# wyhlovecpp/GPT-Image-Edit

Measured on AMD Instinct MI355X. Metric: edited images/sec, 28-step FLUX-Kontext (VAE encode + 28 x MMDiT + VAE decode), higher is better.
Workload: dtype bf16; 1 GPU; cfg2_single_512x512_28step; batch_per_gpu=1, global_batch=1, height=512, width=512, S_txt=512, S_tgt=1024, S_cond=1024, seq_len=2560, num_inference_steps=28, blocks=19 double + 38 single, parallelism=dp1

## Files before the change

### gpt_image_edit_amd/csrc/gemm_epilogue.h

```cpp
#pragma once

#include "mxfp8_quant.h"

constexpr int BM = 256;

struct TileRows {
  int ld, wrap, rpb, b0, r0;
  float inv;
  bool big;
  FK_DEV TileRows(const fk_rows& r, int m0) {
    ld = (int)r.ld;
    if (r.rows_per_batch <= 0) { rpb = 0x7fffffff; wrap = 0; b0 = 0; r0 = 0; big = true; inv = 0.f; }
    else {
      rpb = (int)(r.rows_per_batch > 0x7fffffff ? 0x7fffffff : r.rows_per_batch);
      b0 = (unsigned)m0 / (unsigned)rpb;
      r0 = m0 - b0 * rpb;
      wrap = (int)(r.batch_stride - (int64_t)rpb * r.ld);
      big = rpb >= BM;
      inv = 1.0f / (float)rpb;
    }
  }
  FK_DEV int crossed(int ml) const {
    const int r = r0 + ml;
    const int one = r >= rpb ? 1 : 0;
    const int many = (int)(((float)r + 0.5f) * inv);
    return big ? one : many;
  }
  FK_DEV int off(int ml) const { return ml * ld + crossed(ml) * wrap; }
};

template <int N>
FK_DEV float row_ror(float v) {
  return __int_as_float(__builtin_amdgcn_update_dpp(0, __float_as_int(v), 0x120 + N, 0xf, 0xf, false));
}
FK_DEV float row16_sum(float v) {
  v += row_ror<8>(v);
  v += row_ror<4>(v);
  v += row_ror<2>(v);
  v += row_ror<1>(v);
  return v;
}

FK_DEV int xcd_chunk_index() {
  const int nwg = gridDim.x;
  const int q = nwg >> 3, r = nwg & 7;
  const int xcd = blockIdx.x & 7, idx = blockIdx.x >> 3;
  return (xcd < r ? xcd * (q + 1) : r * (q + 1) + (xcd - r) * q) + idx;
}

template <bool M16>
struct FragMap {
  static FK_DEV int row(int lane, int q) { return M16 ? (q & 1) * 16 + (lane & 15) : (lane & 31); }
  static FK_DEV int col(int lane, int q) { return M16 ? (q >> 1) * 16 + (lane >> 4) * 4 : 8 * q + 4 * (lane >> 5); }
};
FK_DEV f32x4_t quad_get(const f32x16_t& v, int q) { return f32x4_t{v[4 * q], v[4 * q + 1], v[4 * q + 2], v[4 * q + 3]}; }
FK_DEV void quad_set(f32x16_t& v, int q, const f32x4_t& c) {
  v[4 * q] = c[0]; v[4 * q + 1] = c[1]; v[4 * q + 2] = c[2]; v[4 * q + 3] = c[3];
}

template <int EPI, int BN, class C, int HALF = -1, int UB = 8>
FK_DEV void store_tile(const f32x16_t (&acc)[C::NF][C::MF], const fk_gemm_args& p, char* smem, int m0, int n0,
                       int wm, int wn, const u32x4_t* other = nullptr) {
  constexpr int MF0 = HALF > 0 ? C::MF / 2 : 0, MF1 = HALF == 0 ? C::MF / 2 : C::MF;
  constexpr int row0 = HALF > 0 ? BM / 2 : 0;
  int tid = threadIdx.x;
  if constexpr (C::NTHREADS == 256) asm volatile("" : "+v"(tid));
  const int lane = tid & 63;
  using FM = FragMap<C::M16>;
  u32x2_t bw[C::NF][4];
#pragma unroll
  for (int nf = 0; nf < C::NF; ++nf)
#pragma unroll
    for (int q = 0; q < 4; ++q) bw[nf][q] = u32x2_t{0u, 0u};
  if constexpr (EPI != FK_EPI_SCALE) {
    if (p.bias) {
#pragma unroll
      for (int nf = 0; nf < C::NF; ++nf)
#pragma unroll
        for (int q = 0; q < 4; ++q) {
          const int n = n0 + C::tile_col(wn, nf) + FM::col(lane, q);
          bw[nf][q] = *(const u32x2_t*)((const bf16_t*)p.bias + min(n, p.N - 4));
        }
    }
  }
  if constexpr (EPI == FK_EPI_F32DBG) {
#pragma unroll
    for (int nf = 0; nf < C::NF; ++nf)
#pragma unroll
      for (int q = 0; q < 4; ++q) {
        const int n = n0 + C::tile_col(wn, nf) + FM::col(lane, q);
        const float b[4] = {bf_lo(bw[nf][q][0]), bf_hi(bw[nf][q][0]), bf_lo(bw[nf][q][1]), bf_hi(bw[nf][q][1])};
#pragma unroll
        for (int mf = MF0; mf < MF1; ++mf) {
          const int m = m0 + C::tile_row(wm, mf) + FM::row(lane, q);
          f32x4_t x = quad_get(acc[nf][mf], q);
          if constexpr (HALF >= 0) {
#pragma unroll
            for (int j = 0; j < 4; ++j) x[j] += __uint_as_float(other[nf * 2 * C::MF + (mf - MF0) * 4 + q][j]);
          }
          if (m < p.M && n < p.N)
            *(f32x4_t*)((float*)p.C + fk_row_offset(p.c, m) + n) = f32x4_t{x[0] + b[0], x[1] + b[1], x[2] + b[2], x[3] + b[3]};
        }
      }
    return;
  }
  __syncthreads();
  bf16_t* ct = (bf16_t*)smem;
#pragma unroll
  for (int nf = 0; nf < C::NF; ++nf) {
#pragma unroll
    for (int q = 0; q < 4; ++q) {
      const int nl = C::tile_col(wn, nf) + FM::col(lane, q);
      const float b[4] = {bf_lo(bw[nf][q][0]), bf_hi(bw[nf][q][0]), bf_lo(bw[nf][q][1]), bf_hi(bw[nf][q][1])};
#pragma unroll
      for (int mf = MF0; mf < MF1; ++mf) {
        float v[4];
#pragma unroll
        for (int j = 0; j < 4; ++j) {
          float x = acc[nf][mf][q * 4 + j];
          if constexpr (HALF >= 0) x += __uint_as_float(other[nf * 2 * C::MF + (mf - MF0) * 4 + q][j]);
          if constexpr (EPI == FK_EPI_SCALE) v[j] = x * p.alpha;
          else v[j] = x + b[j];
        }
        if constexpr (EPI == FK_EPI_GELU_TANH || EPI == FK_EPI_SILU) {
          round_bf_pair(v[0], v[1]);
          round_bf_pair(v[2], v[3]);
#pragma unroll
          for (int j = 0; j < 4; ++j) v[j] = EPI == FK_EPI_GELU_TANH ? gelu_tanh_f(v[j]) : silu_f(v[j]);
        }
        u32x2_t pk;
        pk[0] = pack_bf2(v[0], v[1]);
        pk[1] = pack_bf2(v[2], v[3]);
        const int ml = C::tile_row(wm, mf) + FM::row(lane, q);
        *(u32x2_t*)(ct + ml * C::CT_LD + nl) = pk;
      }
    }
  }
  __syncthreads();
  constexpr int CPR = BN / 8;
  constexpr int ITERS = (HALF >= 0 ? BM / 2 : BM) * CPR / C::NTHREADS;
  constexpr int U = (EPI == FK_EPI_QKV && (ITERS > 8 || HALF >= 0)) ? 4 : UB;
  static_assert(ITERS % U == 0 && C::NTHREADS % CPR == 0, "epilogue batching");
  const TileRows crow(p.c, m0);
  bf16_t* const cbase = (bf16_t*)p.C + fk_row_offset(p.c, m0);
  const TileRows rrow = (EPI == FK_EPI_GATE_RES || EPI == FK_EPI_RES) ? TileRows(p.r, m0) : crow;
  const bf16_t* const rbase =
      (EPI == FK_EPI_GATE_RES || EPI == FK_EPI_RES) ? (const bf16_t*)p.res + fk_row_offset(p.r, m0) : nullptr;
  fk_rows gr = {0, 0, 0};
  if constexpr (EPI == FK_EPI_GATE_RES) gr.rows_per_batch = p.gate_rows_per_batch;
  const TileRows grow(gr, m0);
  const int D = EPI == FK_EPI_QKV ? p.qkv_heads * 128 : 1;
  const int which = EPI == FK_EPI_QKV ? n0 / D : 0;
  const int cc = tid % CPR, ml0 = row0 + tid / CPR;
  constexpr int ML_STEP = C::NTHREADS / CPR;
  const int n = n0 + cc * 8;
  const int nc = min(n, p.N - 8);
  const int mlast = p.M - 1 - m0;

  if (EPI == FK_EPI_QKV && which < 2) {
    const int hn = n - which * D;
    const int head = hn >> 7, dch = hn & 127;
    const u32x4_t ww = *(const u32x4_t*)((const bf16_t*)(which == 0 ? p.wq : p.wk) + dch);
    bf16_t* const dst = (bf16_t*)(which == 0 ? p.q_out : p.k_out);
#pragma unroll
    for (int j0 = 0; j0 < ITERS; j0 += U) {
      u32x4_t y[U];
      f32x4_t t0[U], t1[U];
      int srow[U], bidx[U];
#pragma unroll
      for (int u = 0; u < U; ++u) {
        const int ml = ml0 + ML_STEP * (j0 + u);
        y[u] = *(const u32x4_t*)(ct + ml * C::CT_LD + cc * 8);
        const int mlc = min(ml, mlast);
        const int nb = crow.crossed(mlc);
        bidx[u] = crow.b0 + nb;
        srow[u] = p.qkv_s_offset + crow.r0 + mlc - nb * crow.rpb;
        const float* tp = p.rope_cs + (int64_t)srow[u] * 128 + dch;
        t0[u] = *(const f32x4_t*)tp;
        t1[u] = *(const f32x4_t*)(tp + 4);
      }
#pragma unroll
      for (int u = 0; u < U; ++u) {
        const int ml = ml0 + ML_STEP * (j0 + u);
        float xv[8];
        float ss = 0.f;
#pragma unroll
        for (int e = 0; e < 4; ++e) {
          xv[2 * e] = bf_lo(y[u][e]);
          xv[2 * e + 1] = bf_hi(y[u][e]);
          ss += xv[2 * e] * xv[2 * e] + xv[2 * e + 1] * xv[2 * e + 1];
        }
        ss = row16_sum(ss);
        const float rs = __builtin_amdgcn_rsqf(ss * (1.0f / 128) + 1e-6f);
        const float cs[4] = {t0[u][0], t0[u][2], t1[u][0], t1[u][2]};
        const float sn[4] = {t0[u][1], t0[u][3], t1[u][1], t1[u][3]};
        u32x4_t ow;
#pragma unroll
        for (int e = 0; e < 4; ++e) {
          float re = xv[2 * e] * rs, im = xv[2 * e + 1] * rs;
          round_bf_pair(re, im);
          re *= bf_lo(ww[e]);
          im *= bf_hi(ww[e]);
          round_bf_pair(re, im);
          const float o0 = __fadd_rn(__fmul_rn(re, cs[e]), __fmul_rn(-im, sn[e]));
          const float o1 = __fadd_rn(__fmul_rn(im, cs[e]), __fmul_rn(re, sn[e]));
          ow[e] = pack_bf2(o0, o1);
        }
        const int hrow = (bidx[u] * p.qkv_heads + head) * p.qkv_s_total + srow[u];
        if (ml <= mlast && n < p.N) *(u32x4_t*)(dst + (int64_t)hrow * 128 + dch) = ow;
      }
    }
    return;
  }

#pragma unroll
  for (int j0 = 0; j0 < ITERS; j0 += U) {
    u32x4_t y[U], rv[U], gv[U];
    int coff[U];
#pragma unroll
    for (int u = 0; u < U; ++u) {
      const int ml = ml0 + ML_STEP * (j0 + u);
      const int mlc = min(ml, mlast);
      y[u] = *(const u32x4_t*)(ct + ml * C::CT_LD + cc * 8);
      coff[u] = crow.off(mlc) + n;
      if constexpr (EPI == FK_EPI_GATE_RES || EPI == FK_EPI_RES) rv[u] = *(const u32x4_t*)(rbase + rrow.off(mlc) + nc);
      if constexpr (EPI == FK_EPI_GATE_RES) {
        const int64_t b = grow.b0 + grow.crossed(mlc);
        gv[u] = *(const u32x4_t*)((const bf16_t*)p.gate + b * p.gate_batch_stride + nc);
      }
    }
#pragma unroll
    for (int u = 0; u < U; ++u) {
      const int ml = ml0 + ML_STEP * (j0 + u);
      u32x4_t o = y[u];
      if constexpr (EPI == FK_EPI_GATE_RES || EPI == FK_EPI_RES) {
#pragma unroll
        for (int e = 0; e < 4; ++e) {
          float y0 = bf_lo(o[e]), y1 = bf_hi(o[e]);
          if constexpr (EPI == FK_EPI_GATE_RES) {
            y0 *= bf_lo(gv[u][e]);
            y1 *= bf_hi(gv[u][e]);
            round_bf_pair(y0, y1);
          }
          o[e] = pack_bf2(bf_lo(rv[u][e]) + y0, bf_hi(rv[u][e]) + y1);
        }
      }
      if (ml <= mlast && n < p.N) *(u32x4_t*)(cbase + coff[u]) = o;
    }
  }
}

template <int EPI, int BN, class C>
FK_DEV void store_tile_mxq(const f32x16_t (&acc)[C::NF][C::MF], const fk_gemm_args& p, uint8_t* __restrict__ q,
                           uint8_t* __restrict__ s, int64_t ldq, int64_t ld_scale, char* smem, int m0, int n0, int wm, int wn) {
  static_assert(EPI == FK_EPI_NONE || EPI == FK_EPI_GELU_TANH, "quantized output: plain and GELU epilogues");
  const int tid = threadIdx.x, lane = tid & 63;
  using FM = FragMap<C::M16>;
  u32x2_t bw[C::NF][4];
#pragma unroll
  for (int nf = 0; nf < C::NF; ++nf)
#pragma unroll
    for (int qd = 0; qd < 4; ++qd) bw[nf][qd] = u32x2_t{0u, 0u};
  if (p.bias) {
#pragma unroll
    for (int nf = 0; nf < C::NF; ++nf)
#pragma unroll
      for (int qd = 0; qd < 4; ++qd) {
        const int n = n0 + C::tile_col(wn, nf) + FM::col(lane, qd);
        bw[nf][qd] = *(const u32x2_t*)((const bf16_t*)p.bias + min(n, p.N - 4));
      }
  }
  __syncthreads();
  bf16_t* ct = (bf16_t*)smem;
#pragma unroll
  for (int nf = 0; nf < C::NF; ++nf) {
#pragma unroll
    for (int qd = 0; qd < 4; ++qd) {
      const int nl = C::tile_col(wn, nf) + FM::col(lane, qd);
      const float b[4] = {bf_lo(bw[nf][qd][0]), bf_hi(bw[nf][qd][0]), bf_lo(bw[nf][qd][1]), bf_hi(bw[nf][qd][1])};
#pragma unroll
      for (int mf = 0; mf < C::MF; ++mf) {
        float v[4];
#pragma unroll
        for (int j = 0; j < 4; ++j) v[j] = acc[nf][mf][qd * 4 + j] + b[j];
        if constexpr (EPI == FK_EPI_GELU_TANH) {
          round_bf_pair(v[0], v[1]);
          round_bf_pair(v[2], v[3]);
#pragma unroll
          for (int j = 0; j < 4; ++j) v[j] = gelu_tanh_f(v[j]);
        }
        u32x2_t pk;
        pk[0] = pack_bf2(v[0], v[1]);
        pk[1] = pack_bf2(v[2], v[3]);
        const int ml = C::tile_row(wm, mf) + FM::row(lane, qd);
        *(u32x2_t*)(ct + ml * C::CT_LD + nl) = pk;
      }
    }
  }
  __syncthreads();
  constexpr int BPR = BN / 32;
  constexpr int ITERS = BM * BPR / C::NTHREADS;
  constexpr int ML_STEP = C::NTHREADS / BPR;
  static_assert(C::NTHREADS % BPR == 0 && (BM * BPR) % C::NTHREADS == 0, "quantized epilogue tiling");
  const int bc = tid % BPR, ml0 = tid / BPR;
  const int mlast = p.M - 1 - m0;
#pragma unroll
  for (int j = 0; j < ITERS; ++j) {
    const int ml = ml0 + ML_STEP * j;
    const u32x4_t* src = (const u32x4_t*)(ct + ml * C::CT_LD + bc * 32);
    uint32_t w[16], out[8];
#pragma unroll
    for (int i = 0; i < 4; ++i) {
      const u32x4_t v = src[i];
      w[4 * i] = v[0]; w[4 * i + 1] = v[1]; w[4 * i + 2] = v[2]; w[4 * i + 3] = v[3];
    }
    const uint32_t sbyte = mx_quant_block(w, out);
    if (ml <= mlast) {
      const int64_t m = (int64_t)m0 + ml;
      u32x4_t* dst = (u32x4_t*)(q + m * ldq + n0 + bc * 32);
      dst[0] = u32x4_t{out[0], out[1], out[2], out[3]};
      dst[1] = u32x4_t{out[4], out[5], out[6], out[7]};
      s[m * ld_scale + (n0 >> 5) + bc] = (uint8_t)sbyte;
    }
  }
}
```

### gpt_image_edit_amd/csrc/gemm_pingpong_bf16.hip

```cpp
#include <stdlib.h>

#include <type_traits>

#include "fk_common.h"

namespace {

#include "gemm_epilogue.h"
#ifndef FK_GROUP_M
#define FK_GROUP_M 8
#endif
constexpr int GROUP_M = FK_GROUP_M;
#ifndef FK_RATE_256
#define FK_RATE_256 1.22
#endif


enum { SK_WHOLE = 0, SK_SYM = 1, SK_SYM_UNANNOUNCED = 2 };

struct GroupArgs {
  fk_gemm_args p[FK_MAX_GROUP];
  int tiles_before[FK_MAX_GROUP + 1];
  int n;
  int big_cols;
  int small_before[FK_MAX_GROUP + 1];
  int xcd_big_start[8], xcd_big_cnt[8], xcd_small_start[8];
  float* sk_partials;
  unsigned* sk_ctl;
  int sk_mode;
  int sk_min_part;
  int group_m;
};

typedef __attribute__((address_space(3))) void lds_void;
typedef __attribute__((address_space(1))) const void gbl_void;

typedef short s16x4_t __attribute__((ext_vector_type(4)));
FK_DEV s16x4_t lds_tr16(const char* p) {
  return __builtin_amdgcn_ds_read_tr16_b64_v4i16((__attribute__((address_space(3))) s16x4_t*)p);
}

FK_DEV void buffer_lds16(__amdgpu_buffer_rsrc_t rsrc, char* lds_dst, int voffset, int soffset) {
#if defined(__HIP_DEVICE_COMPILE__)
  __builtin_amdgcn_raw_ptr_buffer_load_lds(rsrc, (lds_void*)lds_dst, 16, voffset, soffset, 0, 0);
#else
  (void)rsrc; (void)lds_dst; (void)voffset; (void)soffset;
#endif
}

FK_DEV void buffer_lds16(const BufDesc& d, char* lds_dst, int voffset, int soffset) {
  buffer_lds_opaque<16>(d, lds_addr_of(lds_dst), voffset, soffset);
}

template <int N>
FK_DEV void wait_vmcnt() {
  if constexpr (N == 0) asm volatile("s_waitcnt vmcnt(0)" ::: "memory");
  else if constexpr (N == 2) asm volatile("s_waitcnt vmcnt(2)" ::: "memory");
  else if constexpr (N == 4) asm volatile("s_waitcnt vmcnt(4)" ::: "memory");
  else if constexpr (N == 6) asm volatile("s_waitcnt vmcnt(6)" ::: "memory");
  else if constexpr (N == 8) asm volatile("s_waitcnt vmcnt(8)" ::: "memory");
  else if constexpr (N == 10) asm volatile("s_waitcnt vmcnt(10)" ::: "memory");
  else if constexpr (N == 12) asm volatile("s_waitcnt vmcnt(12)" ::: "memory");
  else static_assert(N == 0, "add the vmcnt literal");
}


template <int BN>
FK_DEV void tile_of(const GroupArgs& ga, const int (&before)[FK_MAX_GROUP + 1], int t, int nbn, int col0, int& pi, int& m0,
                    int& n0) {
  pi = 0;
#pragma unroll
  for (int i = 1; i < FK_MAX_GROUP; ++i)
    if (i < ga.n && t >= before[i]) pi = i;
  const fk_gemm_args& p = ga.p[pi];
  t -= before[pi];
  const int nbm = (p.M + BM - 1) / BM;
  const int per_group = ga.group_m * nbn;
  const int g = t / per_group;
  const int first_m = g * ga.group_m;
  const int gm = min(nbm - first_m, ga.group_m);
  const int rem = t - g * per_group;
  m0 = (first_m + rem % gm) * BM;
  n0 = col0 + (rem / gm) * BN;
}
template <int BN>
FK_DEV void select_tile(const GroupArgs& ga, int t, int& pi, int& m0, int& n0) {
  tile_of<BN>(ga, ga.tiles_before, t, (ga.p[0].N + BN - 1) / BN, 0, pi, m0, n0);
}

FK_DEV void mma16_block(f32x16_t& blk, const bf16x8_t& w0, const bf16x8_t& w1, const bf16x8_t& a0, const bf16x8_t& a1) {
  quad_set(blk, 0, __builtin_amdgcn_mfma_f32_16x16x32_bf16(w0, a0, quad_get(blk, 0), 0, 0, 0));
  quad_set(blk, 2, __builtin_amdgcn_mfma_f32_16x16x32_bf16(w1, a0, quad_get(blk, 2), 0, 0, 0));
  quad_set(blk, 1, __builtin_amdgcn_mfma_f32_16x16x32_bf16(w0, a1, quad_get(blk, 1), 0, 0, 0));
  quad_set(blk, 3, __builtin_amdgcn_mfma_f32_16x16x32_bf16(w1, a1, quad_get(blk, 3), 0, 0, 0));
}



template <int BN, bool M16_ = false>
struct Cfg8 {
  static_assert(BN == 256, "the ping-pong kernel is instantiated for the 256 x 256 tile only");
  static constexpr bool M16 = M16_;
  static constexpr int NTHREADS = 512;
  static constexpr int BK = 64, ROW_BYTES = 128;
  static constexpr int WAVES_M = 2, WAVES_N = 4;
  static constexpr int MF = 4, NF = 2;
  static constexpr int HALF_BYTES = 128 * ROW_BYTES;
  static constexpr int BUF_BYTES = 4 * HALF_BYTES;
  static constexpr int RING_BYTES = 2 * BUF_BYTES;
  static constexpr int CT_LD = BN + 8;
  static constexpr int CT_BYTES = BM * CT_LD * 2;
  static constexpr int SMEM_BYTES = RING_BYTES > CT_BYTES ? RING_BYTES : CT_BYTES;
  static FK_DEV int swz(int row) { return (row >> 1) & 7; }
  static FK_DEV int tile_row(int wm, int mf) { return (mf >> 1) * 128 + wm * 64 + (mf & 1) * 32; }
  static FK_DEV int tile_col(int wn, int nf) { return nf * 128 + wn * 32; }
};

template <int EPI, int BN, int LAY = 0, bool M16 = false, bool SYM = false>
FK_DEV void gemm8_body(const GroupArgs& ga, char* smem, int pi, int m0, int n0, int kt_first, int nk, int sk_slot, int sk_part = 0) {
  using C = Cfg8<BN, M16>;
  constexpr bool AT = LAY == 2, WT = LAY >= 1;
  const int tid = threadIdx.x;
  const int lane = tid & 63;
  const int wave = __builtin_amdgcn_readfirstlane(tid >> 6);
  const int wm = wave >> 2, wn = wave & 3;
  const fk_gemm_args& p = ga.p[pi];
  const int kbase = kt_first * (C::BK * 2);

  const int lrow = lane >> 3, slot = lane & 7;
  const int prow = lane >> 4, pslot = lane & 15;
  const __amdgpu_buffer_rsrc_t rs_a = __builtin_amdgcn_make_buffer_rsrc(
      (void*)((const bf16_t*)p.A + (AT ? (int64_t)m0 : fk_row_offset(p.a, m0))), 0, 0x7fffffff, 0x00020000);
  const __amdgpu_buffer_rsrc_t rs_w = __builtin_amdgcn_make_buffer_rsrc(
      (void*)((const bf16_t*)p.W + (WT ? (int64_t)n0 : (int64_t)n0 * p.ldw)), 0, 0x7fffffff, 0x00020000);
  const BufDesc od_a = make_buf_desc((const bf16_t*)p.A + (AT ? (int64_t)m0 : fk_row_offset(p.a, m0)), 0x7fffffffu);
  const BufDesc od_w = make_buf_desc((const bf16_t*)p.W + (WT ? (int64_t)n0 : (int64_t)n0 * p.ldw), 0x7fffffffu);
  int a_voff[2][2], w_voff[2][2];
  {
    const TileRows arow(p.a, m0);
    const int ldw2 = (int)p.ldw * 2, lda2 = (int)p.a.ld * 2;
#pragma unroll
    for (int h = 0; h < 2; ++h)
#pragma unroll
      for (int j = 0; j < 2; ++j) {
        const int rl = h * 128 + (wave * 2 + j) * 8 + lrow;
        const int sw = (slot ^ C::swz(rl)) << 4;
        const int kl = (wave * 2 + j) * 4 + prow;
        const int ct = (h * 128 + (((((pslot >> 2) ^ prow) << 2) | (pslot & 3)) << 3)) * 2;
        a_voff[h][j] = AT ? kl * lda2 + ct : arow.off(min(rl, p.M - 1 - m0)) * 2 + sw;
        w_voff[h][j] = WT ? kl * ldw2 + ct : min(rl, p.N - 1 - n0) * ldw2 + sw;
      }
  }
  const int kstep_a = AT ? C::BK * (int)p.a.ld * 2 : C::BK * 2, kstep_w = WT ? C::BK * (int)p.ldw * 2 : C::BK * 2;
  auto dma_half = [&](int which, int buf, int kt) {
    const int ktc = min(kt, nk - 1);
    char* dst = smem + buf * C::BUF_BYTES + which * C::HALF_BYTES + wave * 2048;
    if (which < 2) {
      const int koff = (AT ? 0 : kbase) + ktc * kstep_a;
      if constexpr (AT || WT) {
        buffer_lds16(od_a, dst, a_voff[which][0], koff);
        buffer_lds16(od_a, dst + 1024, a_voff[which][1], koff);
      } else {
        buffer_lds16(rs_a, dst, a_voff[which][0], koff);
        buffer_lds16(rs_a, dst + 1024, a_voff[which][1], koff);
      }
    } else {
      const int koff = (WT ? 0 : kbase) + ktc * kstep_w;
      if constexpr (AT || WT) {
        buffer_lds16(od_w, dst, w_voff[which - 2][0], koff);
        buffer_lds16(od_w, dst + 1024, w_voff[which - 2][1], koff);
      } else {
        buffer_lds16(rs_w, dst, w_voff[which - 2][0], koff);
        buffer_lds16(rs_w, dst + 1024, w_voff[which - 2][1], koff);
      }
    }
  };

  constexpr int NKS = M16 ? 2 : 4;
  constexpr int ASUB = M16 ? 4 : 2;
  constexpr int WSUB = M16 ? 2 : 1;
  constexpr int SUB_BYTES = (M16 ? 16 : 32) * C::ROW_BYTES;
  const int frow = M16 ? (lane & 15) : (lane & 31), fhalf = M16 ? (lane >> 4) : (lane >> 5), fsw = C::swz(frow);
  int koffs[NKS];
#pragma unroll
  for (int kk = 0; kk < NKS; ++kk) koffs[kk] = ((kk * (M16 ? 4 : 2) + fhalf) ^ fsw) << 4;
  const int a_rd = (wm * 64 + frow) * C::ROW_BYTES;
  const int w_rd = (wn * 32 + frow) * C::ROW_BYTES;

  f32x16_t acc[C::NF][C::MF];
#pragma unroll
  for (int i = 0; i < C::NF; ++i)
#pragma unroll
    for (int j = 0; j < C::MF; ++j)
#pragma unroll
      for (int r = 0; r < 16; ++r) acc[i][j][r] = 0.f;

  bf16x8_t af[ASUB][NKS], wf[2][WSUB][NKS];
  const int tj = (lane & 15) >> 2;
  const int t_lo = M16 ? (8 * (lane >> 4) + tj) * 256 + (lane & 3) * 8
                       : (8 * (lane >> 5) + tj) * 256 + ((lane >> 4) & 1) * 32 + (lane & 3) * 8;
  auto trfrag = [&](const char* half, int kk, int df) {
    const char* vp = M16 ? half + kk * 8192 + (((df >> 1) ^ tj) << 6) + (df & 1) * 32 + t_lo
                         : half + kk * 4096 + ((df ^ tj) << 6) + t_lo;
    const s16x4_t lo = lds_tr16(vp);
    const s16x4_t hi = lds_tr16(vp + 4 * 256);
    bf16x8_t f;
    f[0] = lo[0]; f[1] = lo[1]; f[2] = lo[2]; f[3] = lo[3];
    f[4] = hi[0]; f[5] = hi[1]; f[6] = hi[2]; f[7] = hi[3];
    return f;
  };
  auto read_a = [&](int buf, int h) {
    const char* b = smem + buf * C::BUF_BYTES + h * C::HALF_BYTES;
#pragma unroll
    for (int sub = 0; sub < ASUB; ++sub)
#pragma unroll
      for (int kk = 0; kk < NKS; ++kk) {
        if constexpr (AT) af[sub][kk] = trfrag(b, kk, wm * ASUB + sub);
        else af[sub][kk] = *(const bf16x8_t*)(b + a_rd + sub * SUB_BYTES + koffs[kk]);
      }
  };
  auto read_w = [&](int buf, int j) {
    const char* b = smem + buf * C::BUF_BYTES + (2 + j) * C::HALF_BYTES;
#pragma unroll
    for (int sub = 0; sub < WSUB; ++sub)
#pragma unroll
      for (int kk = 0; kk < NKS; ++kk) {
        if constexpr (WT) wf[j][sub][kk] = trfrag(b, kk, wn * WSUB + sub);
        else wf[j][sub][kk] = *(const bf16x8_t*)(b + w_rd + sub * SUB_BYTES + koffs[kk]);
      }
  };
  auto mma = [&](int i, int j) {
#pragma unroll
    for (int kk = 0; kk < NKS; ++kk)
#pragma unroll
      for (int sub = 0; sub < 2; ++sub) {
        if constexpr (M16) mma16_block(acc[j][2 * i + sub], wf[j][0][kk], wf[j][1][kk], af[2 * sub][kk], af[2 * sub + 1][kk]);
        else acc[j][2 * i + sub] = __builtin_amdgcn_mfma_f32_32x32x16_bf16(wf[j][0][kk], af[sub][kk], acc[j][2 * i + sub], 0, 0, 0);
      }
  };
  auto phase_sync_mma = [&](int i, int j) {
    wait_vmcnt<10>();
    __builtin_amdgcn_sched_barrier(0);
    __builtin_amdgcn_s_barrier();
    asm volatile("s_waitcnt lgkmcnt(0)" ::: "memory");
    __builtin_amdgcn_sched_barrier(0);
    __builtin_amdgcn_s_setprio(1);
    mma(i, j);
    __builtin_amdgcn_s_setprio(0);
    __builtin_amdgcn_sched_barrier(0);
    __builtin_amdgcn_s_barrier();
    __builtin_amdgcn_sched_barrier(0);
  };

  dma_half(2, 0, 0);
  dma_half(0, 0, 0);
  dma_half(3, 0, 0);
  dma_half(1, 0, 0);
  dma_half(2, 1, 1);
  dma_half(0, 1, 1);
  dma_half(3, 1, 1);
  unsigned sk_ann = 0;
  if constexpr (SYM) {
    if (ga.sk_mode != SK_WHOLE && wave == 0) {
      unsigned r = 0;
      if (lane == 0)
        r = __hip_atomic_fetch_add((__attribute__((address_space(1))) unsigned*)(ga.sk_ctl + 2 * (size_t)sk_slot), 1u, __ATOMIC_RELAXED,
                                   __HIP_MEMORY_SCOPE_AGENT);
      sk_ann = __builtin_amdgcn_readfirstlane(r);
    }
  }
  wait_vmcnt<10>();
  __builtin_amdgcn_sched_barrier(0);
  __builtin_amdgcn_s_barrier();
  __builtin_amdgcn_sched_barrier(0);
  read_w(0, 0);
  if (wm == 1) __builtin_amdgcn_s_barrier();
  __builtin_amdgcn_sched_barrier(0);

  auto tile_body = [&](auto bc, int kt) {
    constexpr int b = decltype(bc)::value;
    read_a(b, 0);            dma_half(1, b ^ 1, kt + 1);  phase_sync_mma(0, 0);
    read_w(b, 1);            dma_half(2, b, kt + 2);      phase_sync_mma(0, 1);
    read_a(b, 1);            dma_half(0, b, kt + 2);      phase_sync_mma(1, 0);
    read_w(b ^ 1, 0);        dma_half(3, b, kt + 2);      phase_sync_mma(1, 1);
  };
  for (int kt = 0; kt < nk; kt += 2) {
    tile_body(std::integral_constant<int, 0>{}, kt);
    if (kt + 1 < nk) tile_body(std::integral_constant<int, 1>{}, kt + 1);
  }
  if (wm == 0) __builtin_amdgcn_s_barrier();
  asm volatile("s_waitcnt vmcnt(0)" ::: "memory");

  if (SYM || sk_slot >= 0) {
    typedef __attribute__((address_space(1))) unsigned gu32;
    gu32* const ctl = (gu32*)(ga.sk_ctl + 2 * (size_t)sk_slot);
    const __amdgpu_buffer_rsrc_t rs_p = __builtin_amdgcn_make_buffer_rsrc(
        (void*)(ga.sk_partials + (size_t)sk_slot * (BM * BN)), 0, BM * BN * 4, 0x00020000);
    const bool announced = SYM && ga.sk_mode != SK_WHOLE;
    __syncthreads();
    if (tid == 0) {
      const unsigned t = __hip_atomic_fetch_add(ctl, announced ? 1u : 2u, __ATOMIC_RELAXED, __HIP_MEMORY_SCOPE_AGENT);
      unsigned role;
      if (!announced) role = (t & 2u) ? 1u : 0u;
      else {
        const bool blind = ga.sk_mode == SK_SYM_UNANNOUNCED;
        if ((t & 3u) == 3u) role = (blind || (sk_ann & 3u) == 2u) ? 1u : 2u;
        else role = ((t & 3u) == 2u && !blind) ? 2u : 0u;
      }
      ((volatile unsigned*)smem)[0] = t;
      ((volatile unsigned*)smem)[1] = role;
    }
    __syncthreads();
    const unsigned ticket = __builtin_amdgcn_readfirstlane(((volatile unsigned*)smem)[0]);
    const unsigned role = __builtin_amdgcn_readfirstlane(((volatile unsigned*)smem)[1]);
    const unsigned target = (ticket & ~3u) + 4u;
    auto wait_flag = [&]() {
      if (tid == 0) {
        int spins = 0;
        while (__hip_atomic_load(ctl + 1, __ATOMIC_RELAXED, __HIP_MEMORY_SCOPE_AGENT) != target && spins < (1 << 22)) {
          __builtin_amdgcn_s_sleep(8);
          ++spins;
        }
        __builtin_amdgcn_fence(__ATOMIC_ACQUIRE, "agent");
      }
      __syncthreads();
    };
    auto publish = [&](unsigned step) {
      asm volatile("s_waitcnt vmcnt(0)" ::: "memory");
      __syncthreads();
      if (tid == 0) __hip_atomic_fetch_add(ctl + 1, step, __ATOMIC_RELAXED, __HIP_MEMORY_SCOPE_AGENT);
    };
    constexpr int NV = C::NF * C::MF * 4, NH = NV / 2;
    auto piece_acc = [&](int r) -> f32x16_t& { return acc[(r % NH) / 8][2 * (r / NH) + (r / 4) % 2]; };
    auto store_piece = [&](int r, int at) {
      const f32x16_t& a = piece_acc(r);
      const int q = r & 3;
      const u32x4_t v = {__float_as_uint(a[4 * q]), __float_as_uint(a[4 * q + 1]), __float_as_uint(a[4 * q + 2]),
                         __float_as_uint(a[4 * q + 3])};
      __builtin_amdgcn_raw_buffer_store_b128(v, rs_p, tid * 16, at * (C::NTHREADS * 16),  16);
    };
    auto finish_half = [&](auto keep_c) {
      constexpr int keep = decltype(keep_c)::value;
      u32x4_t other[NH];
#pragma unroll
      for (int r = 0; r < NH; ++r)
        other[r] = __builtin_amdgcn_raw_buffer_load_b128(rs_p, tid * 16, (keep * NH + r) * (C::NTHREADS * 16),  16);
      store_tile<EPI, BN, C, keep>(acc, p, smem, m0, n0, wm, wn, other);
    };
    if constexpr (SYM) {
      if (role == 2u) {
        if (sk_part == 0) {
#pragma unroll
          for (int r = 0; r < NH; ++r) store_piece(NH + r, NH + r);
        } else {
#pragma unroll
          for (int r = 0; r < NH; ++r) store_piece(r, r);
        }
        publish(2u);
        wait_flag();
        if (sk_part == 0) finish_half(std::integral_constant<int, 0>{});
        else finish_half(std::integral_constant<int, 1>{});
        return;
      }
    }
    if (role == 0u) {
#pragma unroll
      for (int r = 0; r < NV; ++r) store_piece(r, r);
      publish(4u);
      return;
    }
    wait_flag();
    if constexpr (SYM) {
      finish_half(std::integral_constant<int, 0>{});
      finish_half(std::integral_constant<int, 1>{});
      return;
    }
#pragma unroll
    for (int r0 = 0; r0 < NV; r0 += 4) {
      u32x4_t v[4];
#pragma unroll
      for (int u = 0; u < 4; ++u)
        v[u] = __builtin_amdgcn_raw_buffer_load_b128(rs_p, tid * 16, (r0 + u) * (C::NTHREADS * 16),  16);
#pragma unroll
      for (int u = 0; u < 4; ++u) {
        f32x16_t& a = piece_acc(r0 + u);
        const int q = u;
#pragma unroll
        for (int j = 0; j < 4; ++j) a[4 * q + j] += __uint_as_float(v[u][j]);
      }
      __builtin_amdgcn_sched_barrier(0);
    }
  }
  store_tile<EPI, BN, C>(acc, p, smem, m0, n0, wm, wn);
}

template <int EPI, int BN, bool SPLITK, int LAY = 0, bool M16 = false>
__global__ __launch_bounds__(512, 2) void gemm8_kernel(const GroupArgs ga) {
  extern __shared__ __attribute__((aligned(16))) char smem[];
  int pi, m0, n0;
  const int t = xcd_chunk_index();
  const int nk_all = ga.p[0].K / Cfg8<BN>::BK;
  if constexpr (SPLITK) {
    select_tile<BN>(ga, t >> 1, pi, m0, n0);
    gemm8_body<EPI, BN, LAY, M16, true>(ga, smem, pi, m0, n0, (t & 1) * (nk_all >> 1), nk_all >> 1, t >> 1, t & 1);
  } else {
    select_tile<BN>(ga, t, pi, m0, n0);
    gemm8_body<EPI, BN, LAY, M16>(ga, smem, pi, m0, n0, 0, nk_all, -1);
  }
}

struct Cfg10 {
  static constexpr bool M16 = true;
  static constexpr int NTHREADS = 256;
  static constexpr int BK = 64, ROW_BYTES = 128;
  static constexpr int MF = 4, NF = 4;
  static constexpr int HALF_BYTES = 128 * ROW_BYTES;
  static constexpr int BUF_BYTES = 4 * HALF_BYTES;
  static constexpr int RING_BYTES = 2 * BUF_BYTES;
  static constexpr int CT_LD = 256 + 8;
  static constexpr int CT_BYTES = BM * CT_LD * 2;
  static constexpr int SMEM_BYTES = RING_BYTES > CT_BYTES ? RING_BYTES : CT_BYTES;
  static FK_DEV int tile_row(int wm, int mf) { return wm * 128 + mf * 32; }
  static FK_DEV int tile_col(int wn, int nf) { return wn * 128 + nf * 32; }
};
typedef int i32x8_t __attribute__((ext_vector_type(8)));
typedef int i32x4_t __attribute__((ext_vector_type(4)));

#define G10_V4(a) "v" #a "0", "v" #a "1", "v" #a "2", "v" #a "3"
#define G10_V10(a) "v" #a "0", "v" #a "1", "v" #a "2", "v" #a "3", "v" #a "4", "v" #a "5", "v" #a "6", "v" #a "7", "v" #a "8", "v" #a "9"
#define G10_CLOBBER_V64_255 \
  "v64", "v65", "v66", "v67", "v68", "v69", G10_V10(7), G10_V10(8), G10_V10(9), G10_V10(10), G10_V10(11), G10_V10(12), G10_V10(13), \
  G10_V10(14), G10_V10(15), G10_V10(16), G10_V10(17), G10_V10(18), G10_V10(19), G10_V10(20), G10_V10(21), G10_V10(22), G10_V10(23), \
  G10_V10(24), "v250", "v251", "v252", "v253", "v254", "v255"
#define G10_OPERANDS \
      : "={a[0:15]}"(acc[0][0]), "={a[16:31]}"(acc[0][1]), "={a[32:47]}"(acc[0][2]), "={a[48:63]}"(acc[0][3]), \
        "={a[64:79]}"(acc[1][0]), "={a[80:95]}"(acc[1][1]), "={a[96:111]}"(acc[1][2]), "={a[112:127]}"(acc[1][3]), \
        "={a[128:143]}"(acc[2][0]), "={a[144:159]}"(acc[2][1]), "={a[160:175]}"(acc[2][2]), "={a[176:191]}"(acc[2][3]), \
        "={a[192:207]}"(acc[3][0]), "={a[208:223]}"(acc[3][1]), "={a[224:239]}"(acc[3][2]), "={a[240:255]}"(acc[3][3]) \
      : "{v[16:23]}"(a_voff), "{v[24:31]}"(w_voff), "{v[32:39]}"(rd), "{v[40:43]}"(wr), "{s[40:43]}"(od_a.w), "{s[44:47]}"(od_w.w), \
        "{s48}"(k0), "{s49}"(nks), "{s50}"(kmax) \
      : "memory", "scc", "s52", "s53", "s54", G10_CLOBBER_V64_255

#define G10_OPERANDS_X \
      : "={a[0:15]}"(acc[0][0]), "={a[16:31]}"(acc[0][1]), "={a[32:47]}"(acc[0][2]), "={a[48:63]}"(acc[0][3]), \
        "={a[64:79]}"(acc[1][0]), "={a[80:95]}"(acc[1][1]), "={a[96:111]}"(acc[1][2]), "={a[112:127]}"(acc[1][3]), \
        "={a[128:143]}"(acc[2][0]), "={a[144:159]}"(acc[2][1]), "={a[160:175]}"(acc[2][2]), "={a[176:191]}"(acc[2][3]), \
        "={a[192:207]}"(acc[3][0]), "={a[208:223]}"(acc[3][1]), "={a[224:239]}"(acc[3][2]), "={a[240:255]}"(acc[3][3]), "={s[56:57]}"(t0), "={s[58:59]}"(t1), "={s[60:61]}"(ta) \
      : "{v[16:23]}"(a_voff), "{v[24:31]}"(w_voff), "{v[32:39]}"(rd), "{v[40:43]}"(wr), "{s[40:43]}"(od_a.w), "{s[44:47]}"(od_w.w), \
        "{s48}"(k0), "{s49}"(nks), "{s50}"(kmax) \
      : "memory", "scc", "s52", "s53", "s54", G10_CLOBBER_V64_255

template <int EPI, int V = 0>
FK_DEV void gemm10_body(const GroupArgs& ga, char* smem, int pi, int m0, int n0, int kt_first, int nk) {
  using C = Cfg10;
#ifdef FK_G10_EXPERIMENTS
  const unsigned long long g10_real0 = __builtin_amdgcn_s_memrealtime(), g10_cyc0 = __builtin_amdgcn_s_memtime();
#endif
  int tid = threadIdx.x;
  asm volatile("" : "+v"(tid));
  const int lane = tid & 63;
  const int wave = __builtin_amdgcn_readfirstlane(tid >> 6);
  const int wm = wave >> 1, wn = wave & 1;
  const fk_gemm_args& p = ga.p[pi];
  const BufDesc od_a = make_buf_desc((const bf16_t*)p.A + fk_row_offset(p.a, m0), 0x7fffffffu);
  const BufDesc od_w = make_buf_desc((const bf16_t*)p.W + (int64_t)n0 * p.ldw, 0x7fffffffu);
  const int lrow = lane >> 3, chunk = lane & 7;
  i32x8_t a_voff, w_voff;
  {
    const TileRows arow(p.a, m0);
    const int ldw2 = (int)p.ldw * 2;
#pragma unroll
    for (int i = 0; i < 8; ++i) {
      const int rl = wave * 64 + i * 8 + lrow;
      a_voff[i] = arow.off(min(rl, p.M - 1 - m0)) * 2 + chunk * 16;
      w_voff[i] = min(rl, p.N - 1 - n0) * ldw2 + chunk * 16;
    }
  }
  const int base = (int)lds_addr_of(smem);
  i32x8_t rd;
  i32x4_t wr;
  {
    const int frow = lane & 15, fhalf = lane >> 4, fsw = (frow >> 1) & 7;
#pragma unroll
    for (int buf = 0; buf < 2; ++buf)
#pragma unroll
      for (int kk = 0; kk < 2; ++kk) {
        const int ko = ((kk * 4 + fhalf) ^ fsw) << 4;
        rd[2 * buf + kk] = base + buf * C::BUF_BYTES + wm * C::HALF_BYTES + frow * C::ROW_BYTES + ko;
        rd[4 + 2 * buf + kk] = base + buf * C::BUF_BYTES + (2 + wn) * C::HALF_BYTES + frow * C::ROW_BYTES + ko;
      }
#pragma unroll
    for (int buf = 0; buf < 2; ++buf)
#pragma unroll
      for (int par = 0; par < 2; ++par)
        wr[2 * buf + par] = base + buf * C::BUF_BYTES + (wave >> 1) * C::HALF_BYTES + (wave & 1) * 8192 + lrow * C::ROW_BYTES +
                            ((chunk ^ ((par * 4 + (lrow >> 1)) & 7)) << 4);
  }
  const int k0 = __builtin_amdgcn_readfirstlane(kt_first * (C::BK * 2));
  const int nks = __builtin_amdgcn_readfirstlane(nk);
  const int kmax = k0 + (nks - 1) * (C::BK * 2);

  f32x16_t acc[C::NF][C::MF];
  if constexpr (V == 0) {
    asm volatile(
#include "gemm10_loop.inc"
        G10_OPERANDS);
  }
#ifdef FK_G10_EXPERIMENTS
  unsigned long long t0 = 0, t1 = 0, ta = 0;
  (void)t0; (void)t1; (void)ta;
  if constexpr (V == 1) { asm volatile(
#include "gemm10_loop_x1.inc"
        G10_OPERANDS_X); }
  else if constexpr (V == 2) { asm volatile(
#include "gemm10_loop_x2.inc"
        G10_OPERANDS_X); }
  else if constexpr (V == 3) { asm volatile(
#include "gemm10_loop_x3.inc"
        G10_OPERANDS_X); }
  else if constexpr (V == 4) { asm volatile(
#include "gemm10_loop_x4.inc"
        G10_OPERANDS_X); }
  else if constexpr (V == 5) { asm volatile(
#include "gemm10_loop_x5.inc"
        G10_OPERANDS_X); }
  else if constexpr (V == 6) { asm volatile(
#include "gemm10_loop_x6.inc"
        G10_OPERANDS_X); }
  else if constexpr (V == 7) { asm volatile(
#include "gemm10_loop_x7.inc"
        G10_OPERANDS_X); }
  else if constexpr (V == 8) { asm volatile(
#include "gemm10_loop_x8.inc"
        G10_OPERANDS_X); }
  else if constexpr (V == 9) { asm volatile(
#include "gemm10_loop_x9.inc"
        G10_OPERANDS_X); }
  else if constexpr (V == 10) { asm volatile(
#include "gemm10_loop_x10.inc"
        G10_OPERANDS_X); }
  else if constexpr (V == 11) { asm volatile(
#include "gemm10_loop_x11.inc"
        G10_OPERANDS_X); }
  else if constexpr (V == 12) { asm volatile(
#include "gemm10_loop_x12.inc"
        G10_OPERANDS_X); }
  else if constexpr (V == 13) { asm volatile(
#include "gemm10_loop_x13.inc"
        G10_OPERANDS_X); }
  else if constexpr (V == 14) { asm volatile(
#include "gemm10_loop_x14.inc"
        G10_OPERANDS_X); }
  else if constexpr (V == 15) { asm volatile(
#include "gemm10_loop_x15.inc"
        G10_OPERANDS_X); }
  else if constexpr (V == 16) { asm volatile(
#include "gemm10_loop_x16.inc"
        G10_OPERANDS_X); }
  else if constexpr (V == 17) { asm volatile(
#include "gemm10_loop_x17.inc"
        G10_OPERANDS_X); }
  else if constexpr (V == 18) { asm volatile(
#include "gemm10_loop_x18.inc"
        G10_OPERANDS_X); }
  else if constexpr (V == 19) { asm volatile(
#include "gemm10_loop_x19.inc"
        G10_OPERANDS_X); }
  else if constexpr (V == 20) { asm volatile(
#include "gemm10_loop_x20.inc"
        G10_OPERANDS_X); }
#endif
  store_tile<EPI, 256, C>(acc, p, smem, m0, n0, wm, wn);
#ifdef FK_G10_EXPERIMENTS
  if constexpr (V > 0) {
    if (tid == 0) {
      unsigned long long* rec = (unsigned long long*)((bf16_t*)p.C + (int64_t)p.M * p.c.ld) + (size_t)blockIdx.x * 8;
      rec[0] = (unsigned long long)__builtin_amdgcn_s_getreg(63492) | ((unsigned long long)__builtin_amdgcn_s_getreg(63508) << 32);
      rec[1] = g10_real0; rec[2] = __builtin_amdgcn_s_memrealtime();
      rec[3] = g10_cyc0; rec[4] = t0; rec[5] = t1; rec[6] = __builtin_amdgcn_s_memtime();
      rec[7] = ta;
    }
  }
#endif
}

template <int EPI, int V = 0, bool PERSIST = false>
__global__ __launch_bounds__(256, 1) void gemm10_kernel(const GroupArgs ga) {
  extern __shared__ __attribute__((aligned(16))) char smem[];
  const int nk = ga.p[0].K / Cfg10::BK;
  if constexpr (PERSIST) {
    const int total = ga.tiles_before[FK_MAX_GROUP];
    for (int t = xcd_chunk_index(); t < total; t += gridDim.x) {
      int pi, m0, n0;
      select_tile<256>(ga, t, pi, m0, n0);
      gemm10_body<EPI, V>(ga, smem, pi, m0, n0, 0, nk);
      asm volatile("s_waitcnt lgkmcnt(0)\n\ts_barrier" ::: "memory");
    }
  } else {
    int pi, m0, n0;
    select_tile<256>(ga, xcd_chunk_index(), pi, m0, n0);
    gemm10_body<EPI, V>(ga, smem, pi, m0, n0, 0, nk);
  }
}

template <int EPI, int BN, bool M16 = false>
__global__ __launch_bounds__(512, 2) void gemm8_streamk_kernel(const GroupArgs ga) {
  extern __shared__ __attribute__((aligned(16))) char smem[];
  const int pos = xcd_chunk_index();
  const unsigned G = gridDim.x, nk = ga.p[0].K / Cfg8<BN>::BK;
  const unsigned U = (unsigned)ga.tiles_before[FK_MAX_GROUP] * nk, qU = U / G, rU = U - qU * G;
  auto cut = [&](unsigned j) __attribute__((always_inline)) {
    unsigned c = qU * j + (rU * j) / G;
    const unsigned r = c % nk;
    if (r != 0 && r < (unsigned)ga.sk_min_part) c -= r;
    else if (r != 0 && nk - r < (unsigned)ga.sk_min_part) c += nk - r;
    return (int)c;
  };
  const int u = cut(pos);
  int u_end = cut(pos + 1);
  while (u < u_end) {
    const int t = (unsigned)(u_end - 1) / nk;
    const int k1 = u_end - t * (int)nk, k0 = max(u - t * (int)nk, 0);
    u_end -= k1 - k0;
    int pi, m0, n0;
    select_tile<BN>(ga, t, pi, m0, n0);
    const bool part = k0 > 0 || k1 < (int)nk;
    gemm8_body<EPI, BN, 0, M16>(ga, smem, pi, m0, n0, k0, k1 - k0, part ? (k1 < (int)nk ? pos + 1 : pos) : -1);
    __syncthreads();
  }
}

template <int BN>
int count_tiles(GroupArgs& ga, const fk_gemm_args* probs, int n) {
  int total = 0;
  for (int i = 0; i < FK_MAX_GROUP; ++i) {
    ga.tiles_before[i] = total;
    if (i < n) total += ((probs[i].M + BM - 1) / BM) * ((probs[i].N + BN - 1) / BN);
  }
  ga.tiles_before[FK_MAX_GROUP] = total;
  return total;
}

template <int EPI, int BN, bool SPLITK, int LAY = 0, bool M16 = false>
int launch8(GroupArgs& ga, const fk_gemm_args* probs, int n, hipStream_t stream) {
  const int total = count_tiles<BN>(ga, probs, n);
  auto kern = gemm8_kernel<EPI, BN, SPLITK, LAY, M16>;
  FK_ENSURE_MAX_LDS(kern, Cfg8<BN>::SMEM_BYTES, "fk_gemm_bf16 (256 x 256 tile, 8 waves ping-pong)");
  hipLaunchKernelGGL(kern, dim3(SPLITK ? 2 * total : total), dim3(512), Cfg8<BN>::SMEM_BYTES, stream, ga);
  FK_CHECK_LAUNCH("fk_gemm_bf16 (256 x 256 tile, 8 waves ping-pong)");
  return FK_OK;
}

template <int EPI, int BN, bool M16 = false>
int launch8_streamk(GroupArgs& ga, const fk_gemm_args* probs, int n, int grid, hipStream_t stream) {
  count_tiles<BN>(ga, probs, n);
  auto kern = gemm8_streamk_kernel<EPI, BN, M16>;
  FK_ENSURE_MAX_LDS(kern, Cfg8<BN>::SMEM_BYTES, "fk_gemm_bf16 (256 x 256 tile, stream-K ranges)");
  hipLaunchKernelGGL(kern, dim3(grid), dim3(512), Cfg8<BN>::SMEM_BYTES, stream, ga);
  FK_CHECK_LAUNCH("fk_gemm_bf16 (256 x 256 tile, stream-K ranges)");
  return FK_OK;
}


int cu_count();
template <int EPI>
int launch10(GroupArgs& ga, const fk_gemm_args* probs, int n, hipStream_t stream) {
  const int total = count_tiles<256>(ga, probs, n);
#ifdef FK_G10_EXPERIMENTS
  if constexpr (EPI == FK_EPI_NONE) {
    static const int x = getenv("FK_G10_X") ? atoi(getenv("FK_G10_X")) : 0;
    static const int persist = getenv("FK_G10_PERSIST") ? atoi(getenv("FK_G10_PERSIST")) : 0;
    void (*kx)(const GroupArgs) = nullptr;
    if (persist) kx = x == 1 ? gemm10_kernel<EPI, 1, true> : gemm10_kernel<EPI, 0, true>;
    else switch (x) {
      case 1: kx = gemm10_kernel<EPI, 1>; break;
      case 2: kx = gemm10_kernel<EPI, 2>; break;
      case 3: kx = gemm10_kernel<EPI, 3>; break;
      case 4: kx = gemm10_kernel<EPI, 4>; break;
      case 5: kx = gemm10_kernel<EPI, 5>; break;
      case 6: kx = gemm10_kernel<EPI, 6>; break;
      case 7: kx = gemm10_kernel<EPI, 7>; break;
      case 8: kx = gemm10_kernel<EPI, 8>; break;
      case 9: kx = gemm10_kernel<EPI, 9>; break;
      case 10: kx = gemm10_kernel<EPI, 10>; break;
      case 11: kx = gemm10_kernel<EPI, 11>; break;
      case 12: kx = gemm10_kernel<EPI, 12>; break;
      case 13: kx = gemm10_kernel<EPI, 13>; break;
      case 14: kx = gemm10_kernel<EPI, 14>; break;
      case 15: kx = gemm10_kernel<EPI, 15>; break;
      case 16: kx = gemm10_kernel<EPI, 16>; break;
      case 17: kx = gemm10_kernel<EPI, 17>; break;
      case 18: kx = gemm10_kernel<EPI, 18>; break;
      case 19: kx = gemm10_kernel<EPI, 19>; break;
      case 20: kx = gemm10_kernel<EPI, 20>; break;
      default: break;
    }
    if (kx) {
      if (hipFuncSetAttribute((const void*)kx, hipFuncAttributeMaxDynamicSharedMemorySize, Cfg10::SMEM_BYTES) != hipSuccess) return FK_EINVAL;
      hipLaunchKernelGGL(kx, dim3(persist ? (total < cu_count() ? total : cu_count()) : total), dim3(256), Cfg10::SMEM_BYTES, stream, ga);
      FK_CHECK_LAUNCH("fk_gemm_bf16 (gemm10 experiment)");
      return FK_OK;
    }
  }
#endif
  const int G = cu_count();
  if (total >= 4 * G) {
    auto kern = gemm10_kernel<EPI, 0, true>;
    FK_ENSURE_MAX_LDS(kern, Cfg10::SMEM_BYTES, "fk_gemm_bf16 (256 x 256 tile, 4 waves, hand-placed loop, one workgroup per CU)");
    hipLaunchKernelGGL(kern, dim3(G), dim3(256), Cfg10::SMEM_BYTES, stream, ga);
    FK_CHECK_LAUNCH("fk_gemm_bf16 (256 x 256 tile, 4 waves, hand-placed loop, one workgroup per CU)");
    return FK_OK;
  }
  auto kern = gemm10_kernel<EPI, 0, false>;
  FK_ENSURE_MAX_LDS(kern, Cfg10::SMEM_BYTES, "fk_gemm_bf16 (256 x 256 tile, 4 waves, hand-placed loop)");
  hipLaunchKernelGGL(kern, dim3(total), dim3(256), Cfg10::SMEM_BYTES, stream, ga);
  FK_CHECK_LAUNCH("fk_gemm_bf16 (256 x 256 tile, 4 waves, hand-placed loop)");
  return FK_OK;
}

template <int BN, bool M16_ = false>
struct Cfg9 {
  static_assert(BN == 128, "instantiated for the 256 x 128 tile only");
  static constexpr bool M16 = M16_;
  static constexpr int NTHREADS = 512;
  static constexpr int BK = 64, ROW_BYTES = 128;
  static constexpr int WAVES_M = 4, WAVES_N = 2;
  static constexpr int WTM = 64, WTN = 64, MF = 2, NF = 2;
  static constexpr int A_HALF = 128 * ROW_BYTES, W_PART = 64 * ROW_BYTES;
  static constexpr int STAGE_BYTES = 2 * A_HALF + 2 * W_PART;
  static constexpr int STAGES = 3;
  static constexpr int CT_LD = BN + 8;
  static constexpr int CT_BYTES = BM * CT_LD * 2;
  static constexpr int SMEM_BYTES = STAGES * STAGE_BYTES > CT_BYTES ? STAGES * STAGE_BYTES : CT_BYTES;
  static FK_DEV int swz(int row) { return (row >> 1) & 7; }
  static FK_DEV int tile_row(int wm, int mf) { return wm * WTM + mf * 32; }
  static FK_DEV int tile_col(int wn, int nf) { return wn * WTN + nf * 32; }
};

template <int EPI, int BN, bool M16 = false>
FK_DEV void gemm9_body(const GroupArgs& ga, char* smem, int pi, int m0, int n0) {
  using C = Cfg9<BN, M16>;
  const int tid = threadIdx.x;
  const int lane = tid & 63;
  const int wave = __builtin_amdgcn_readfirstlane(tid >> 6);
  const int wm = wave & 3, wn = wave >> 2;
  const fk_gemm_args& p = ga.p[pi];
  const int nk = p.K / C::BK;

  const int lrow = lane >> 3, slot = lane & 7;
  const __amdgpu_buffer_rsrc_t rs_a =
      __builtin_amdgcn_make_buffer_rsrc((void*)((const bf16_t*)p.A + fk_row_offset(p.a, m0)), 0, 0x7fffffff, 0x00020000);
  const __amdgpu_buffer_rsrc_t rs_w =
      __builtin_amdgcn_make_buffer_rsrc((void*)((const bf16_t*)p.W + (int64_t)n0 * p.ldw), 0, 0x7fffffff, 0x00020000);
  int a_voff[2][2], w_voff[2];
  {
    const TileRows arow(p.a, m0);
    const int ldw2 = (int)p.ldw * 2;
#pragma unroll
    for (int h = 0; h < 2; ++h)
#pragma unroll
      for (int j = 0; j < 2; ++j) {
        const int rl = h * 128 + (wave * 2 + j) * 8 + lrow;
        a_voff[h][j] = arow.off(min(rl, p.M - 1 - m0)) * 2 + ((slot ^ C::swz(rl)) << 4);
      }
#pragma unroll
    for (int j = 0; j < 2; ++j) {
      const int sr = wave * 8 + lrow;
      const int rl = (sr >> 5) * 64 + j * 32 + (sr & 31);
      w_voff[j] = min(rl, p.N - 1 - n0) * ldw2 + ((slot ^ C::swz(sr)) << 4);
    }
  }
  auto dma_a = [&](int stage, int kt) {
    const int koff = min(kt, nk - 1) * (C::BK * 2);
    char* dst = smem + stage * C::STAGE_BYTES + wave * 2048;
    buffer_lds16(rs_a, dst, a_voff[0][0], koff);
    buffer_lds16(rs_a, dst + 1024, a_voff[0][1], koff);
    buffer_lds16(rs_a, dst + C::A_HALF, a_voff[1][0], koff);
    buffer_lds16(rs_a, dst + C::A_HALF + 1024, a_voff[1][1], koff);
  };
  auto dma_w = [&](int j, int stage, int kt) {
    const int koff = min(kt, nk - 1) * (C::BK * 2);
    buffer_lds16(rs_w, smem + stage * C::STAGE_BYTES + 2 * C::A_HALF + j * C::W_PART + wave * 1024, w_voff[j], koff);
  };

  constexpr int NKS = M16 ? 2 : 4, ASUB = M16 ? 4 : 2, WSUB = M16 ? 2 : 1;
  constexpr int SUB_BYTES = (M16 ? 16 : 32) * C::ROW_BYTES;
  const int frow = M16 ? (lane & 15) : (lane & 31), fhalf = M16 ? (lane >> 4) : (lane >> 5), fsw = C::swz(frow);
  int koffs[NKS];
#pragma unroll
  for (int kk = 0; kk < NKS; ++kk) koffs[kk] = ((kk * (M16 ? 4 : 2) + fhalf) ^ fsw) << 4;
  const int a_rd = (wm * 64 + frow) * C::ROW_BYTES;
  const int w_rd = 2 * C::A_HALF + (wn * 32 + frow) * C::ROW_BYTES;

  f32x16_t acc[C::NF][C::MF];
#pragma unroll
  for (int i = 0; i < C::NF; ++i)
#pragma unroll
    for (int j = 0; j < C::MF; ++j)
#pragma unroll
      for (int r = 0; r < 16; ++r) acc[i][j][r] = 0.f;

  bf16x8_t af[ASUB][NKS], wf[2][WSUB][NKS];
  auto read_a = [&](int stage) {
    const char* b = smem + stage * C::STAGE_BYTES + a_rd;
#pragma unroll
    for (int sub = 0; sub < ASUB; ++sub)
#pragma unroll
      for (int kk = 0; kk < NKS; ++kk) af[sub][kk] = *(const bf16x8_t*)(b + sub * SUB_BYTES + koffs[kk]);
  };
  auto read_w = [&](int stage, int j) {
    const char* b = smem + stage * C::STAGE_BYTES + w_rd + j * C::W_PART;
#pragma unroll
    for (int sub = 0; sub < WSUB; ++sub)
#pragma unroll
      for (int kk = 0; kk < NKS; ++kk) wf[j][sub][kk] = *(const bf16x8_t*)(b + sub * SUB_BYTES + koffs[kk]);
  };
  auto mma = [&](int j) {
#pragma unroll
    for (int kk = 0; kk < NKS; ++kk)
#pragma unroll
      for (int mf = 0; mf < 2; ++mf) {
        if constexpr (M16) mma16_block(acc[j][mf], wf[j][0][kk], wf[j][1][kk], af[2 * mf][kk], af[2 * mf + 1][kk]);
        else acc[j][mf] = __builtin_amdgcn_mfma_f32_32x32x16_bf16(wf[j][0][kk], af[mf][kk], acc[j][mf], 0, 0, 0);
      }
  };
  auto phase_sync_mma = [&](auto vm, int j) {
    wait_vmcnt<decltype(vm)::value>();
    __builtin_amdgcn_sched_barrier(0);
    __builtin_amdgcn_s_barrier();
    asm volatile("s_waitcnt lgkmcnt(0)" ::: "memory");
    __builtin_amdgcn_sched_barrier(0);
    __builtin_amdgcn_s_setprio(1);
    mma(j);
    __builtin_amdgcn_s_setprio(0);
    __builtin_amdgcn_sched_barrier(0);
    __builtin_amdgcn_s_barrier();
    __builtin_amdgcn_sched_barrier(0);
  };
  using V10 = std::integral_constant<int, 10>;
  using V8 = std::integral_constant<int, 8>;

  dma_w(0, 0, 0);
  dma_a(0, 0);
  dma_w(1, 0, 0);
  dma_w(0, 1, 1);
  dma_a(1, 1);
  dma_w(1, 1, 1);
  dma_w(0, 2, 2);
  wait_vmcnt<8>();
  __builtin_amdgcn_sched_barrier(0);
  __builtin_amdgcn_s_barrier();
  __builtin_amdgcn_sched_barrier(0);
  read_w(0, 0);
  if (wn == 1) __builtin_amdgcn_s_barrier();
  __builtin_amdgcn_sched_barrier(0);

  auto tile_body = [&](auto sc, int kt) {
    constexpr int st = decltype(sc)::value, st1 = (st + 1) % 3, st2 = (st + 2) % 3;
    read_a(st);                        dma_a(st2, kt + 2);                             phase_sync_mma(V10{}, 0);
    read_w(st, 1); read_w(st1, 0);     dma_w(0, st, kt + 3); dma_w(1, st2, kt + 2);    phase_sync_mma(V8{}, 1);
  };
  for (int kt = 0; kt < nk; kt += 3) {
    tile_body(std::integral_constant<int, 0>{}, kt);
    if (kt + 1 < nk) tile_body(std::integral_constant<int, 1>{}, kt + 1);
    if (kt + 2 < nk) tile_body(std::integral_constant<int, 2>{}, kt + 2);
  }
  if (wn == 0) __builtin_amdgcn_s_barrier();
  asm volatile("s_waitcnt vmcnt(0)" ::: "memory");

  store_tile<EPI, BN, C>(acc, p, smem, m0, n0, wm, wn);
}

template <int EPI, int BN, bool M16 = false>
__global__ __launch_bounds__(512, 2) void gemm9_kernel(const GroupArgs ga) {
  extern __shared__ __attribute__((aligned(16))) char smem[];
  int pi, m0, n0;
  select_tile<BN>(ga, xcd_chunk_index(), pi, m0, n0);
  gemm9_body<EPI, BN, M16>(ga, smem, pi, m0, n0);
}

template <int EPI, int BN, bool M16 = false>
int launch9(GroupArgs& ga, const fk_gemm_args* probs, int n, hipStream_t stream) {
  const int total = count_tiles<BN>(ga, probs, n);
  auto kern = gemm9_kernel<EPI, BN, M16>;
  FK_ENSURE_MAX_LDS(kern, Cfg9<BN>::SMEM_BYTES, "fk_gemm_bf16 (256 x 128 tile, 8 waves ping-pong)");
  hipLaunchKernelGGL(kern, dim3(total), dim3(512), Cfg9<BN>::SMEM_BYTES, stream, ga);
  FK_CHECK_LAUNCH("fk_gemm_bf16 (256 x 128 tile, 8 waves ping-pong)");
  return FK_OK;
}

template <int EPI, bool M16 = false>
__global__ __launch_bounds__(512, 2) void gemm_mix_kernel(const GroupArgs ga) {
  extern __shared__ __attribute__((aligned(16))) char smem[];
  const int xcd = blockIdx.x & 7, idx = blockIdx.x >> 3;
  const int nbig = ga.xcd_big_cnt[xcd];
  int pi, m0, n0;
  if (idx < nbig) {
    tile_of<256>(ga, ga.tiles_before, ga.xcd_big_start[xcd] + idx, ga.big_cols, 0, pi, m0, n0);
    gemm8_body<EPI, 256, 0, M16>(ga, smem, pi, m0, n0, 0, ga.p[0].K / 64, -1);
  } else {
    tile_of<128>(ga, ga.small_before, ga.xcd_small_start[xcd] + idx - nbig, (ga.p[0].N - ga.big_cols * 256 + 127) / 128,
                 ga.big_cols * 256, pi, m0, n0);
    gemm9_body<EPI, 128, M16>(ga, smem, pi, m0, n0);
  }
}

constexpr int MIX_SMEM = Cfg8<256>::SMEM_BYTES > Cfg9<128>::SMEM_BYTES ? Cfg8<256>::SMEM_BYTES : Cfg9<128>::SMEM_BYTES;

template <int EPI, bool M16 = false>
int launch_mix(GroupArgs& ga, const fk_gemm_args* probs, int n, int big_cols, hipStream_t stream) {
  const int ncols128 = (probs[0].N - big_cols * 256 + 127) / 128;
  int tb = 0, ts = 0;
  for (int i = 0; i < FK_MAX_GROUP; ++i) {
    ga.tiles_before[i] = tb;
    ga.small_before[i] = ts;
    if (i < n) {
      const int nbm = (probs[i].M + BM - 1) / BM;
      tb += nbm * big_cols;
      ts += nbm * ncols128;
    }
  }
  ga.tiles_before[FK_MAX_GROUP] = tb;
  ga.small_before[FK_MAX_GROUP] = ts;
  ga.big_cols = big_cols;
  const int W = tb + ts;
  int bs = 0, ss = 0;
  for (int x = 0; x < 8; ++x) {
    const int wx = W / 8 + (x < W % 8 ? 1 : 0), bx = tb / 8 + (x < tb % 8 ? 1 : 0);
    if (wx < bx) return FK_E2BIG_STRIDES;
    ga.xcd_big_start[x] = bs;
    ga.xcd_big_cnt[x] = bx;
    ga.xcd_small_start[x] = ss;
    bs += bx;
    ss += wx - bx;
  }
  auto kern = gemm_mix_kernel<EPI, M16>;
  FK_ENSURE_MAX_LDS(kern, MIX_SMEM, "fk_gemm_bf16 (mixed 256 x 256 / 256 x 128 tiles)");
  hipLaunchKernelGGL(kern, dim3(W), dim3(512), MIX_SMEM, stream, ga);
  FK_CHECK_LAUNCH("fk_gemm_bf16 (mixed 256 x 256 / 256 x 128 tiles)");
  return FK_OK;
}

template <int EPI, bool M16>
int launch_variant_m(GroupArgs& ga, const fk_gemm_args* probs, int n, int variant, int big_cols, hipStream_t stream) {
  switch (variant) {
    case 256: return launch8<EPI, 256, false, 0, M16>(ga, probs, n, stream);
    case 384: return launch_mix<EPI, M16>(ga, probs, n, big_cols, stream);
    case 512: return launch8<EPI, 256, true, 0, M16>(ga, probs, n, stream);
    case 640: return launch8_streamk<EPI, 256, M16>(ga, probs, n, big_cols, stream);
    case 1024: return launch10<EPI>(ga, probs, n, stream);
    default: return launch9<EPI, 128, M16>(ga, probs, n, stream);
  }
}
template <int EPI>
int launch_variant(GroupArgs& ga, const fk_gemm_args* probs, int n, int variant, int big_cols, bool m16, hipStream_t stream) {
  return m16 ? launch_variant_m<EPI, true>(ga, probs, n, variant, big_cols, stream)
             : launch_variant_m<EPI, false>(ga, probs, n, variant, big_cols, stream);
}

int cu_count() {
  static int cus = 0;
  if (!cus) {
    int dev = 0, v = 0;
    if (hipGetDevice(&dev) == hipSuccess &&
        hipDeviceGetAttribute(&v, hipDeviceAttributeMultiprocessorCount, dev) == hipSuccess && v > 0) cus = v;
    else return 256;
  }
  return cus;
}

double makespan(long nb, long ns, double cs, int G) {
  const long full = nb / G, rem = nb % G;
  double ta = (double)full, tb = (double)full + 1.0, end = rem ? tb : ta;
  const long na = G - rem;
  if (nb == 0) end = 0.0;
  while (ns > 0) {
    if (rem == 0 || ta <= tb) {
      const long k = ns < na ? ns : na;
      ta += cs; ns -= k;
      if (ta > end) end = ta;
    } else {
      const long k = ns < rem ? ns : rem;
      tb += cs; ns -= k;
      if (tb > end) end = tb;
    }
  }
  return end;
}

struct Plan { int variant, big_cols; };
constexpr int SK_MIN_PART = 16;
constexpr double SK_TAIL_WHOLE = 17.0e-6, SK_TAIL_SYM = 9.0e-6;
#ifndef FK_SPLITK_SYMMETRIC_DEFAULT
#define FK_SPLITK_SYMMETRIC_DEFAULT 1
#endif
constexpr int SK_MODE_DEFAULT = FK_SPLITK_SYMMETRIC_DEFAULT ? SK_SYM : SK_WHOLE;

Plan plan_launch(long nbm, int N, int K, int G, int allow, bool have_ws, int ws_slots, int sk_mode) {
  const double c128 = 0.5 * FK_RATE_256;
  const long t128 = nbm * ((N + 127) / 128), t256 = nbm * ((N + 255) / 256);
  Plan best = {128, 0};
  double tbest = makespan(0, t128, c128, G);
  if (N % 256 != 0) return best;
  const double t_256 = makespan(t256, 0, c128, G);
  if (t_256 < tbest) { tbest = t_256; best = {256, 0}; }
  if (allow & 1) {
    const int nb256 = N / 256;
    for (int cb = 1; cb < nb256; ++cb) {
      const long ts = nbm * 2 * (nb256 - cb);
      if (ts < 8) continue;
      const double t = makespan(nbm * cb, ts, c128, G);
      if (t < tbest * 0.97) { tbest = t; best = {384, cb}; }
    }
  }
  if ((allow & 2) && have_ws && K >= 6144 && (K / 64) % 4 == 0 && 2 * t256 <= G && t256 <= ws_slots) {
    const double t = 0.5 + (sk_mode == SK_WHOLE ? SK_TAIL_WHOLE : SK_TAIL_SYM) / (K * 25.8e-9);
    if (t < tbest * 0.97) { tbest = t; best = {512, 0}; }
  }
  if ((allow & 4) && have_ws && K >= 6144 && t256 > G && G <= ws_slots &&
      t256 * (K / 64) >= (long)G * (K / 64 + 2 * SK_MIN_PART) && t256 * (long)(K / 64) < (1l << 31)) {
    const double t = (double)t256 / G + SK_TAIL_WHOLE / (K * 25.8e-9);
    if (t < tbest * 0.97) { tbest = t; best = {640, G}; }
  }
  return best;
}
}

static inline void report_variant(const fk_gemm_args* probs, int v) {
  if (probs[0].variant_used) *probs[0].variant_used = v;
}

#ifndef FK_GEMM_MFMA_DEFAULT
#define FK_GEMM_MFMA_DEFAULT 16
#endif
constexpr int GEMM_MFMA_DEFAULT = FK_GEMM_MFMA_DEFAULT;

int fk_gemm2_launch(const fk_gemm_args* probs, int n, int variant_hint, hipStream_t stream) {
  const fk_gemm_args& ctl = probs[0];
  if (variant_hint == 0) variant_hint = ctl.variant;
  if (!(variant_hint == 0 || variant_hint == 128 || variant_hint == 256 || variant_hint == 384 || variant_hint == 512 || variant_hint == 640 ||
        variant_hint == 1024)) {
    fk_set_error("fk_gemm_bf16: variant %d is not one of 0 (launch plan), 128, 256, 384 (mixed), 512 (split-K pairs), 640 (stream-K ranges), "
                 "1024 (4-wave hand-placed 256 x 256 kernel)", variant_hint);
    return FK_EINVAL;
  }
  constexpr int SK_BITS = FK_GEMM_PLAN_SPLITK_WHOLE | FK_GEMM_PLAN_SPLITK_SYMMETRIC | FK_GEMM_PLAN_SPLITK_UNANNOUNCED;
  const int sk_bits = ctl.plan & SK_BITS;
  if (ctl.plan != 0 && (ctl.plan & ~(15 | SK_BITS)) != 0 || (ctl.plan != 0 && !(ctl.plan & FK_GEMM_PLAN_EXPLICIT)) ||
      (sk_bits & (sk_bits - 1)) != 0) {
    fk_set_error("fk_gemm_bf16: plan %d is not 0 (default) or FK_GEMM_PLAN_EXPLICIT | allow bits 0..2 | at most one "
                 "FK_GEMM_PLAN_SPLITK_* exchange", ctl.plan);
    return FK_EINVAL;
  }
  if (ctl.group_m < 0 || ctl.group_m > 4096 || !(ctl.mfma == 0 || ctl.mfma == 16 || ctl.mfma == 32)) {
    fk_set_error("fk_gemm_bf16: group_m %d must be 0 (default) or 1..4096, mfma %d one of 0 / 16 / 32", ctl.group_m, ctl.mfma);
    return FK_EINVAL;
  }
  const int plan_allow = ctl.plan ? (ctl.plan & 7) : 3;
  const int sk_mode = sk_bits == FK_GEMM_PLAN_SPLITK_WHOLE ? SK_WHOLE : sk_bits == FK_GEMM_PLAN_SPLITK_SYMMETRIC ? SK_SYM
                      : sk_bits == FK_GEMM_PLAN_SPLITK_UNANNOUNCED ? SK_SYM_UNANNOUNCED : SK_MODE_DEFAULT;
  GroupArgs ga;
  ga.sk_mode = sk_mode;
  ga.n = n;
  ga.group_m = ctl.group_m ? ctl.group_m : GROUP_M;
  ga.big_cols = 0;
  ga.sk_partials = nullptr;
  ga.sk_ctl = nullptr;
  long nbm_total = 0;
  bool ok256 = probs[0].N % 256 == 0, ok32 = true;
  for (int i = 0; i < FK_MAX_GROUP; ++i) {
    ga.p[i] = probs[i < n ? i : 0];
    if (i < n) {
      nbm_total += (probs[i].M + BM - 1) / BM;
      auto span = [](const fk_rows& r) {
        const long long ld = r.ld < 0 ? -r.ld : r.ld, bs = r.batch_stride < 0 ? -r.batch_stride : r.batch_stride;
        return (BM * ld + (r.rows_per_batch > 0 ? bs : 0)) * 2;
      };
      if ((long long)BM * probs[i].ldw * 2 >= (1ll << 31) || probs[i].ldw < 0) ok32 = false;
      const bool has_res = probs[i].epilogue == FK_EPI_GATE_RES || probs[i].epilogue == FK_EPI_RES;
      const fk_rows* ops[3] = {&probs[i].a, &probs[i].c, has_res ? &probs[i].r : nullptr};
      for (const fk_rows* r : ops) {
        if (!r) continue;
        if (span(*r) >= (1ll << 31) || r->ld < 0) ok32 = false;
        if (r->rows_per_batch > 0 && r->batch_stride < r->rows_per_batch * r->ld) ok32 = false;
      }
    }
  }
  if (!ok32) return FK_E2BIG_STRIDES;

  const int lay = probs[0].layout;
  if (lay != 0) {
    for (int i = 0; i < n; ++i) {
      const fk_gemm_args& q = probs[i];
      const bool uniform_a = q.a.rows_per_batch <= 0 || q.a.batch_stride == q.a.rows_per_batch * q.a.ld;
      if (q.layout != lay || q.N % 256 != 0 || q.K % 64 != 0 || q.ldw % 8 != 0 || (int64_t)q.K * q.ldw * 2 >= (1ll << 31) ||
          (lay == 2 && (q.M % 256 != 0 || !uniform_a || q.a.ld % 8 != 0 || (int64_t)q.K * q.a.ld * 2 >= (1ll << 31))) ||
          (q.epilogue != FK_EPI_NONE && !(lay == 1 && q.epilogue == FK_EPI_RES))) {
        fk_set_error("fk_gemm_bf16: layout %d needs N %% 256 == 0, K %% 64 == 0%s, epilogue none%s and operands below 2 GiB "
                     "(M %d N %d K %d epilogue %d)", lay, lay == 2 ? ", M % 256 == 0, uniformly strided A rows" : "",
                     lay == 1 ? " / residual" : "", q.M, q.N, q.K, q.epilogue);
        return FK_EUNSUPPORTED;
      }
    }
    report_variant(probs, 256);
    static const bool km32 = getenv("FK_KMAJOR_MFMA") && atoi(getenv("FK_KMAJOR_MFMA")) == 32;
    if (!km32 && (ctl.mfma ? ctl.mfma : GEMM_MFMA_DEFAULT) == 16) {
      if (lay == 1 && probs[0].epilogue == FK_EPI_RES) return launch8<FK_EPI_RES, 256, false, 1, true>(ga, probs, n, stream);
      if (lay == 1) return launch8<FK_EPI_NONE, 256, false, 1, true>(ga, probs, n, stream);
      if (lay == 2) return launch8<FK_EPI_NONE, 256, false, 2, true>(ga, probs, n, stream);
    }
    if (lay == 1 && probs[0].epilogue == FK_EPI_RES) return launch8<FK_EPI_RES, 256, false, 1>(ga, probs, n, stream);
    if (lay == 1) return launch8<FK_EPI_NONE, 256, false, 1>(ga, probs, n, stream);
    if (lay == 2) return launch8<FK_EPI_NONE, 256, false, 2>(ga, probs, n, stream);
    fk_set_error("fk_gemm_bf16: unknown layout %d", lay);
    return FK_EUNSUPPORTED;
  }

  const int ws_slots = probs[0].splitk_ws ? probs[0].splitk_slots : 0;
  const int N = probs[0].N, K = probs[0].K;
  const int G = cu_count();
  const long t256 = nbm_total * ((N + 255) / 256);
  const bool sk_ok = ws_slots > 0 && ok256 && (K / 64) % 4 == 0 && t256 <= ws_slots;
  Plan plan;
  switch (variant_hint) {
    case 128: plan = {128, 0}; break;
    case 256: plan = {ok256 ? 256 : 128, 0}; break;
    case 384: {
      plan = plan_launch(nbm_total, N, K, G, 1, false, 0, sk_mode);
      if (plan.variant != 384) {
        plan = {128, 0};
        if (ok256 && N >= 512) {
          double tb = 1e30;
          for (int cb = 1; cb < N / 256; ++cb) {
            if (nbm_total * 2 * (N / 256 - cb) < 8) continue;
            const double t = makespan(nbm_total * cb, nbm_total * 2 * (N / 256 - cb), 0.5 * FK_RATE_256, G);
            if (t < tb) { tb = t; plan = {384, cb}; }
          }
        }
      }
      break;
    }
    case 512: plan = {sk_ok ? 512 : (ok256 ? 256 : 128), 0}; break;
    case 1024: plan = {ok256 ? 1024 : 128, 0}; break;
    case 640: {
      const int Gs = G < ws_slots ? G : ws_slots;
      const bool ok = ws_slots > 0 && ok256 && t256 * (K / 64) >= (long)Gs * (K / 64 + 2 * SK_MIN_PART) && t256 * (long)(K / 64) < (1l << 31);
      plan = ok ? Plan{640, Gs} : Plan{ok256 ? 256 : 128, 0};
      break;
    }
    default: plan = plan_launch(nbm_total, N, K, G, plan_allow, ws_slots > 0 && ok256, ws_slots, sk_mode); break;
  }
  ga.sk_min_part = SK_MIN_PART;
  if (plan.variant == 512 || plan.variant == 640) {
    ga.sk_partials = (float*)probs[0].splitk_ws;
    ga.sk_ctl = (unsigned*)((char*)probs[0].splitk_ws + (size_t)ws_slots * (BM * 256 * 4));
  }
  const bool m16 = (ctl.mfma ? ctl.mfma : GEMM_MFMA_DEFAULT) == 16;
  static const bool g10_auto = !(getenv("FK_GEMM10") && atoi(getenv("FK_GEMM10")) == 0);
  if (plan.variant == 256 && variant_hint == 0 && m16 && g10_auto && K >= 6144 && t256 >= 4L * G) plan.variant = 1024;
  report_variant(probs, plan.variant);
  int rc;
  switch (probs[0].out_fp32 == 2 ? FK_EPI_F32DBG : probs[0].epilogue) {
    case FK_EPI_F32DBG: rc = launch_variant<FK_EPI_F32DBG>(ga, probs, n, plan.variant, plan.big_cols, m16, stream); break;
    case FK_EPI_NONE: rc = launch_variant<FK_EPI_NONE>(ga, probs, n, plan.variant, plan.big_cols, m16, stream); break;
    case FK_EPI_GELU_TANH: rc = launch_variant<FK_EPI_GELU_TANH>(ga, probs, n, plan.variant, plan.big_cols, m16, stream); break;
    case FK_EPI_SILU: rc = launch_variant<FK_EPI_SILU>(ga, probs, n, plan.variant, plan.big_cols, m16, stream); break;
    case FK_EPI_GATE_RES: rc = launch_variant<FK_EPI_GATE_RES>(ga, probs, n, plan.variant, plan.big_cols, m16, stream); break;
    case FK_EPI_RES: rc = launch_variant<FK_EPI_RES>(ga, probs, n, plan.variant, plan.big_cols, m16, stream); break;
    case FK_EPI_SCALE: rc = launch_variant<FK_EPI_SCALE>(ga, probs, n, plan.variant, plan.big_cols, m16, stream); break;
    case FK_EPI_QKV: rc = launch_variant<FK_EPI_QKV>(ga, probs, n, plan.variant, plan.big_cols, m16, stream); break;
    default: fk_set_error("fk_gemm_bf16: unknown epilogue %d", probs[0].epilogue); return FK_EUNSUPPORTED;
  }
  if (rc == FK_E2BIG_STRIDES && plan.variant == 384) {
    report_variant(probs, 128);
    return fk_gemm2_launch(probs, n, 128, stream);
  }
  return rc;
}
```

Baseline: 1.082 images/s.

## Precompute GEMM tile maps on host and issue prologue loads before epilogue args

Moves tile-to-problem mapping into a host-precomputed table that uses magic-number division, and pins those values in scalar registers so each workgroup decodes its tile cheaply. Adds per-problem flat-row flags so that A/C/residual addressing skips the batch-wrap arithmetic when rows are contiguous. The first DMA prefetches are issued before the full argument struct and the split-K atomic are touched, which shortens the kernel entry latency. In exchange it adds optional timestamp instrumentation and extra host-side setup, and it carries some risk of regressions in edge cases of the mapping.

```diff
diff --git a/gpt_image_edit_amd/csrc/gemm_epilogue.h b/gpt_image_edit_amd/csrc/gemm_epilogue.h
--- a/gpt_image_edit_amd/csrc/gemm_epilogue.h
+++ b/gpt_image_edit_amd/csrc/gemm_epilogue.h
@@ -6,15 +6,17 @@
 
 struct TileRows {
   int ld, wrap, rpb, b0, r0;
+  int rf;
   float inv;
   bool big;
-  FK_DEV TileRows(const fk_rows& r, int m0) {
+  FK_DEV TileRows(const fk_rows& r, int m0, bool flat = false) {
     ld = (int)r.ld;
-    if (r.rows_per_batch <= 0) { rpb = 0x7fffffff; wrap = 0; b0 = 0; r0 = 0; big = true; inv = 0.f; }
+    if (flat) { rpb = 0x7fffffff; wrap = 0; b0 = 0; r0 = rf = m0; big = true; inv = 0.f; }
+    else if (r.rows_per_batch <= 0) { rpb = 0x7fffffff; wrap = 0; b0 = 0; r0 = 0; rf = m0; big = true; inv = 0.f; }
     else {
       rpb = (int)(r.rows_per_batch > 0x7fffffff ? 0x7fffffff : r.rows_per_batch);
       b0 = (unsigned)m0 / (unsigned)rpb;
-      r0 = m0 - b0 * rpb;
+      r0 = rf = m0 - b0 * rpb;
       wrap = (int)(r.batch_stride - (int64_t)rpb * r.ld);
       big = rpb >= BM;
       inv = 1.0f / (float)rpb;
@@ -27,6 +29,9 @@
     return big ? one : many;
   }
   FK_DEV int off(int ml) const { return ml * ld + crossed(ml) * wrap; }
+  FK_DEV int64_t first(const fk_rows& r) const {
+    return (int64_t)b0 * r.batch_stride + (int64_t)rf * r.ld;
+  }
 };
 
 template <int N>
@@ -60,7 +65,7 @@
 
 template <int EPI, int BN, class C, int HALF = -1, int UB = 8>
 FK_DEV void store_tile(const f32x16_t (&acc)[C::NF][C::MF], const fk_gemm_args& p, char* smem, int m0, int n0,
-                       int wm, int wn, const u32x4_t* other = nullptr) {
+                       int wm, int wn, const u32x4_t* other = nullptr, int flat = 0) {
   constexpr int MF0 = HALF > 0 ? C::MF / 2 : 0, MF1 = HALF == 0 ? C::MF / 2 : C::MF;
   constexpr int row0 = HALF > 0 ? BM / 2 : 0;
   int tid = threadIdx.x;
@@ -141,14 +146,15 @@
   constexpr int ITERS = (HALF >= 0 ? BM / 2 : BM) * CPR / C::NTHREADS;
   constexpr int U = (EPI == FK_EPI_QKV && (ITERS > 8 || HALF >= 0)) ? 4 : UB;
   static_assert(ITERS % U == 0 && C::NTHREADS % CPR == 0, "epilogue batching");
-  const TileRows crow(p.c, m0);
-  bf16_t* const cbase = (bf16_t*)p.C + fk_row_offset(p.c, m0);
-  const TileRows rrow = (EPI == FK_EPI_GATE_RES || EPI == FK_EPI_RES) ? TileRows(p.r, m0) : crow;
-  const bf16_t* const rbase =
-      (EPI == FK_EPI_GATE_RES || EPI == FK_EPI_RES) ? (const bf16_t*)p.res + fk_row_offset(p.r, m0) : nullptr;
+  constexpr bool HAS_RES = EPI == FK_EPI_GATE_RES || EPI == FK_EPI_RES;
+  const bool cflat = flat & 2, rflat = flat & 4, gflat = flat & 8;
+  const TileRows crow(p.c, m0, cflat);
+  bf16_t* const cbase = (bf16_t*)p.C + crow.first(p.c);
+  const TileRows rrow = HAS_RES ? TileRows(p.r, m0, rflat) : crow;
+  const bf16_t* const rbase = HAS_RES ? (const bf16_t*)p.res + rrow.first(p.r) : nullptr;
   fk_rows gr = {0, 0, 0};
   if constexpr (EPI == FK_EPI_GATE_RES) gr.rows_per_batch = p.gate_rows_per_batch;
-  const TileRows grow(gr, m0);
+  const TileRows grow(gr, m0, gflat);
   const int D = EPI == FK_EPI_QKV ? p.qkv_heads * 128 : 1;
   const int which = EPI == FK_EPI_QKV ? n0 / D : 0;
   const int cc = tid % CPR, ml0 = row0 + tid / CPR;
diff --git a/gpt_image_edit_amd/csrc/gemm_pingpong_bf16.hip b/gpt_image_edit_amd/csrc/gemm_pingpong_bf16.hip
--- a/gpt_image_edit_amd/csrc/gemm_pingpong_bf16.hip
+++ b/gpt_image_edit_amd/csrc/gemm_pingpong_bf16.hip
@@ -7,6 +7,9 @@
 namespace {
 
 #include "gemm_epilogue.h"
+#define FK_TM_FN __host__ __device__ __forceinline__
+#include "gemm_tile_map.h"
+static_assert(TM_MAX_GROUP == FK_MAX_GROUP && TM_BM == BM, "gemm_tile_map.h mirrors fk.h / gemm_epilogue.h");
 #ifndef FK_GROUP_M
 #define FK_GROUP_M 8
 #endif
@@ -19,18 +22,35 @@
 enum { SK_WHOLE = 0, SK_SYM = 1, SK_SYM_UNANNOUNCED = 2 };
 
 struct GroupArgs {
+  TileEntry e;
+  ProbEntry pe[FK_MAX_GROUP];
   fk_gemm_args p[FK_MAX_GROUP];
-  int tiles_before[FK_MAX_GROUP + 1];
-  int n;
-  int big_cols;
-  int small_before[FK_MAX_GROUP + 1];
-  int xcd_big_start[8], xcd_big_cnt[8], xcd_small_start[8];
   float* sk_partials;
   unsigned* sk_ctl;
   int sk_mode;
   int sk_min_part;
-  int group_m;
 };
+
+
+#ifdef FK_ENTRY_STAMPS
+__device__ unsigned long long* fk_entry_stamp_buf = nullptr;
+struct EntryStamps {
+  unsigned long long t[5];
+  template <int I> FK_DEV void mark() { t[I] = __builtin_amdgcn_s_memtime(); }
+  FK_DEV void flush() const {
+    if (threadIdx.x == 0 && fk_entry_stamp_buf) {
+      unsigned long long* r = fk_entry_stamp_buf + (size_t)blockIdx.x * 8;
+      for (int i = 0; i < 5; ++i) r[i] = t[i];
+      r[5] = (unsigned long long)__builtin_amdgcn_s_getreg(63492) | ((unsigned long long)__builtin_amdgcn_s_getreg(63508) << 32);
+    }
+  }
+};
+#else
+struct EntryStamps {
+  template <int I> FK_DEV void mark() {}
+  FK_DEV void flush() const {}
+};
+#endif
 
 typedef __attribute__((address_space(3))) void lds_void;
 typedef __attribute__((address_space(1))) const void gbl_void;
@@ -65,27 +85,51 @@
 }
 
 
+struct Hot {
+  TmHot h;
+  uint32_t xq, xr, grid;
+  int nk;
+};
+#define FK_PIN_CLASS(h)                                                                                                   \
+  "+s"((h).before[0]), "+s"((h).before[1]), "+s"((h).before[2]), "+s"((h).nbm[0]), "+s"((h).nbm[1]), "+s"((h).nbm[2]),       \
+      "+s"((h).nbm[3]), "+s"((h).last_mul[0]), "+s"((h).last_mul[1]), "+s"((h).last_mul[2]), "+s"((h).last_mul[3]),          \
+      "+s"((h).per_group), "+s"((h).col0), "+s"((h).per_group_mul), "+s"((h).group_m_mul)
+#define FK_PIN_HEAD(x) "+s"((x).h.n), "+s"((x).h.group_m), "+s"((x).xq), "+s"((x).xr), "+s"((x).grid), "+s"((x).nk)
+FK_DEV Hot load_hot(const GroupArgs& ga) {
+  Hot x;
+  x.h = tm_hot(ga.e, ga.e.cls[0]);
+  x.xq = ga.e.xq; x.xr = ga.e.xr; x.grid = ga.e.grid; x.nk = ga.e.nk;
+  asm volatile("" : FK_PIN_HEAD(x), FK_PIN_CLASS(x.h));
+  return x;
+}
+FK_DEV ProbEntry load_prob(const GroupArgs& ga, int pi) {
+  ProbEntry q = ga.pe[pi];
+  asm volatile("" : "+s"(q.A), "+s"(q.W), "+s"(q.lda), "+s"(q.ldw), "+s"(q.M), "+s"(q.N), "+s"(q.K), "+s"(q.flags));
+  return q;
+}
 template <int BN>
-FK_DEV void tile_of(const GroupArgs& ga, const int (&before)[FK_MAX_GROUP + 1], int t, int nbn, int col0, int& pi, int& m0,
-                    int& n0) {
-  pi = 0;
-#pragma unroll
-  for (int i = 1; i < FK_MAX_GROUP; ++i)
-    if (i < ga.n && t >= before[i]) pi = i;
-  const fk_gemm_args& p = ga.p[pi];
-  t -= before[pi];
-  const int nbm = (p.M + BM - 1) / BM;
-  const int per_group = ga.group_m * nbn;
-  const int g = t / per_group;
-  const int first_m = g * ga.group_m;
-  const int gm = min(nbm - first_m, ga.group_m);
-  const int rem = t - g * per_group;
-  m0 = (first_m + rem % gm) * BM;
-  n0 = col0 + (rem / gm) * BN;
-}
-template <int BN>
-FK_DEV void select_tile(const GroupArgs& ga, int t, int& pi, int& m0, int& n0) {
-  tile_of<BN>(ga, ga.tiles_before, t, (ga.p[0].N + BN - 1) / BN, 0, pi, m0, n0);
+FK_DEV void select_tile(const Hot& x, int t, int& pi, int& m0, int& n0) { tm_tile_hot(x.h, BN, t, pi, m0, n0); }
+FK_DEV int xcd_chunk_of(const Hot& x) { return tm_xcd_chunk(x.xq, x.xr, blockIdx.x); }
+
+FK_DEV int behind_requests(int pi) {
+  pi = __builtin_amdgcn_readfirstlane(pi);
+  asm volatile("" : "+s"(pi) :: "memory");
+  return pi;
+}
+
+template <int NR>
+FK_DEV int64_t tile_a_rows(const GroupArgs& ga, int pi, const ProbEntry& q, int m0, const int (&rl)[NR], int (&off)[NR]) {
+#pragma unroll
+  for (int i = 0; i < NR; ++i) off[i] = min(rl[i], q.M - 1 - m0) * q.lda;
+  int64_t first = (int64_t)m0 * q.lda;
+  if (__builtin_expect(!(q.flags & TM_A_FLAT), 0)) {
+    const fk_rows& a = ga.p[pi].a;
+    const TileRows arow(a, m0);
+#pragma unroll
+    for (int i = 0; i < NR; ++i) off[i] = arow.off(min(rl[i], q.M - 1 - m0));
+    first = arow.first(a);
+  }
+  return first;
 }
 
 FK_DEV void mma16_block(f32x16_t& blk, const bf16x8_t& w0, const bf16x8_t& w1, const bf16x8_t& a0, const bf16x8_t& a1) {
@@ -117,41 +161,47 @@
 };
 
 template <int EPI, int BN, int LAY = 0, bool M16 = false, bool SYM = false>
-FK_DEV void gemm8_body(const GroupArgs& ga, char* smem, int pi, int m0, int n0, int kt_first, int nk, int sk_slot, int sk_part = 0) {
+FK_DEV void gemm8_body(const GroupArgs& ga, char* smem, int pi, int m0, int n0, int kt_first, int nk, int sk_slot, int sk_part = 0, EntryStamps* st = nullptr) {
+  EntryStamps st_none;
+  if (!st) st = &st_none;
   using C = Cfg8<BN, M16>;
   constexpr bool AT = LAY == 2, WT = LAY >= 1;
   const int tid = threadIdx.x;
   const int lane = tid & 63;
   const int wave = __builtin_amdgcn_readfirstlane(tid >> 6);
   const int wm = wave >> 2, wn = wave & 3;
-  const fk_gemm_args& p = ga.p[pi];
+  const ProbEntry q = load_prob(ga, pi);
   const int kbase = kt_first * (C::BK * 2);
 
   const int lrow = lane >> 3, slot = lane & 7;
   const int prow = lane >> 4, pslot = lane & 15;
-  const __amdgpu_buffer_rsrc_t rs_a = __builtin_amdgcn_make_buffer_rsrc(
-      (void*)((const bf16_t*)p.A + (AT ? (int64_t)m0 : fk_row_offset(p.a, m0))), 0, 0x7fffffff, 0x00020000);
-  const __amdgpu_buffer_rsrc_t rs_w = __builtin_amdgcn_make_buffer_rsrc(
-      (void*)((const bf16_t*)p.W + (WT ? (int64_t)n0 : (int64_t)n0 * p.ldw)), 0, 0x7fffffff, 0x00020000);
-  const BufDesc od_a = make_buf_desc((const bf16_t*)p.A + (AT ? (int64_t)m0 : fk_row_offset(p.a, m0)), 0x7fffffffu);
-  const BufDesc od_w = make_buf_desc((const bf16_t*)p.W + (WT ? (int64_t)n0 : (int64_t)n0 * p.ldw), 0x7fffffffu);
   int a_voff[2][2], w_voff[2][2];
+  int64_t a_first = m0;
   {
-    const TileRows arow(p.a, m0);
-    const int ldw2 = (int)p.ldw * 2, lda2 = (int)p.a.ld * 2;
+    const int ldw2 = q.ldw * 2, lda2 = q.lda * 2;
+    int rls[4], aoff[4] = {0, 0, 0, 0};
+#pragma unroll
+    for (int i = 0; i < 4; ++i) rls[i] = (i >> 1) * 128 + (wave * 2 + (i & 1)) * 8 + lrow;
+    if constexpr (!AT) a_first = tile_a_rows<4>(ga, pi, q, m0, rls, aoff);
 #pragma unroll
     for (int h = 0; h < 2; ++h)
 #pragma unroll
       for (int j = 0; j < 2; ++j) {
-        const int rl = h * 128 + (wave * 2 + j) * 8 + lrow;
+        const int rl = rls[h * 2 + j];
         const int sw = (slot ^ C::swz(rl)) << 4;
         const int kl = (wave * 2 + j) * 4 + prow;
         const int ct = (h * 128 + (((((pslot >> 2) ^ prow) << 2) | (pslot & 3)) << 3)) * 2;
-        a_voff[h][j] = AT ? kl * lda2 + ct : arow.off(min(rl, p.M - 1 - m0)) * 2 + sw;
-        w_voff[h][j] = WT ? kl * ldw2 + ct : min(rl, p.N - 1 - n0) * ldw2 + sw;
-      }
-  }
-  const int kstep_a = AT ? C::BK * (int)p.a.ld * 2 : C::BK * 2, kstep_w = WT ? C::BK * (int)p.ldw * 2 : C::BK * 2;
+        a_voff[h][j] = AT ? kl * lda2 + ct : aoff[h * 2 + j] * 2 + sw;
+        w_voff[h][j] = WT ? kl * ldw2 + ct : min(rl, q.N - 1 - n0) * ldw2 + sw;
+      }
+  }
+  const bf16_t* const a_src = (const bf16_t*)q.A + a_first;
+  const bf16_t* const w_src = (const bf16_t*)q.W + (WT ? (int64_t)n0 : (int64_t)n0 * q.ldw);
+  const __amdgpu_buffer_rsrc_t rs_a = __builtin_amdgcn_make_buffer_rsrc((void*)a_src, 0, 0x7fffffff, 0x00020000);
+  const __amdgpu_buffer_rsrc_t rs_w = __builtin_amdgcn_make_buffer_rsrc((void*)w_src, 0, 0x7fffffff, 0x00020000);
+  const BufDesc od_a = make_buf_desc(a_src, 0x7fffffffu);
+  const BufDesc od_w = make_buf_desc(w_src, 0x7fffffffu);
+  const int kstep_a = AT ? C::BK * q.lda * 2 : C::BK * 2, kstep_w = WT ? C::BK * q.ldw * 2 : C::BK * 2;
   auto dma_half = [&](int which, int buf, int kt) {
     const int ktc = min(kt, nk - 1);
     char* dst = smem + buf * C::BUF_BYTES + which * C::HALF_BYTES + wave * 2048;
@@ -175,6 +225,26 @@
       }
     }
   };
+
+  dma_half(2, 0, 0);
+  st->mark<1>();
+  dma_half(0, 0, 0);
+  dma_half(3, 0, 0);
+  dma_half(1, 0, 0);
+  dma_half(2, 1, 1);
+  dma_half(0, 1, 1);
+  dma_half(3, 1, 1);
+  const fk_gemm_args& p = ga.p[behind_requests(pi)];
+  unsigned sk_ann = 0;
+  if constexpr (SYM) {
+    if (ga.sk_mode != SK_WHOLE && wave == 0) {
+      unsigned r = 0;
+      if (lane == 0)
+        r = __hip_atomic_fetch_add((__attribute__((address_space(1))) unsigned*)(ga.sk_ctl + 2 * (size_t)sk_slot), 1u, __ATOMIC_RELAXED,
+                                   __HIP_MEMORY_SCOPE_AGENT);
+      sk_ann = __builtin_amdgcn_readfirstlane(r);
+    }
+  }
 
   constexpr int NKS = M16 ? 2 : 4;
   constexpr int ASUB = M16 ? 4 : 2;
@@ -252,23 +322,6 @@
     __builtin_amdgcn_sched_barrier(0);
   };
 
-  dma_half(2, 0, 0);
-  dma_half(0, 0, 0);
-  dma_half(3, 0, 0);
-  dma_half(1, 0, 0);
-  dma_half(2, 1, 1);
-  dma_half(0, 1, 1);
-  dma_half(3, 1, 1);
-  unsigned sk_ann = 0;
-  if constexpr (SYM) {
-    if (ga.sk_mode != SK_WHOLE && wave == 0) {
-      unsigned r = 0;
-      if (lane == 0)
-        r = __hip_atomic_fetch_add((__attribute__((address_space(1))) unsigned*)(ga.sk_ctl + 2 * (size_t)sk_slot), 1u, __ATOMIC_RELAXED,
-                                   __HIP_MEMORY_SCOPE_AGENT);
-      sk_ann = __builtin_amdgcn_readfirstlane(r);
-    }
-  }
   wait_vmcnt<10>();
   __builtin_amdgcn_sched_barrier(0);
   __builtin_amdgcn_s_barrier();
@@ -276,6 +329,7 @@
   read_w(0, 0);
   if (wm == 1) __builtin_amdgcn_s_barrier();
   __builtin_amdgcn_sched_barrier(0);
+  st->mark<2>();
 
   auto tile_body = [&](auto bc, int kt) {
     constexpr int b = decltype(bc)::value;
@@ -288,6 +342,7 @@
     tile_body(std::integral_constant<int, 0>{}, kt);
     if (kt + 1 < nk) tile_body(std::integral_constant<int, 1>{}, kt + 1);
   }
+  st->mark<3>();
   if (wm == 0) __builtin_amdgcn_s_barrier();
   asm volatile("s_waitcnt vmcnt(0)" ::: "memory");
 
@@ -345,7 +400,7 @@
 #pragma unroll
       for (int r = 0; r < NH; ++r)
         other[r] = __builtin_amdgcn_raw_buffer_load_b128(rs_p, tid * 16, (keep * NH + r) * (C::NTHREADS * 16),  16);
-      store_tile<EPI, BN, C, keep>(acc, p, smem, m0, n0, wm, wn, other);
+      store_tile<EPI, BN, C, keep>(acc, p, smem, m0, n0, wm, wn, other, q.flags);
     };
     if constexpr (SYM) {
       if (role == 2u) {
@@ -391,22 +446,27 @@
       __builtin_amdgcn_sched_barrier(0);
     }
   }
-  store_tile<EPI, BN, C>(acc, p, smem, m0, n0, wm, wn);
+  store_tile<EPI, BN, C>(acc, p, smem, m0, n0, wm, wn, nullptr, q.flags);
 }
 
 template <int EPI, int BN, bool SPLITK, int LAY = 0, bool M16 = false>
 __global__ __launch_bounds__(512, 2) void gemm8_kernel(const GroupArgs ga) {
   extern __shared__ __attribute__((aligned(16))) char smem[];
+  EntryStamps st;
+  st.mark<0>();
   int pi, m0, n0;
-  const int t = xcd_chunk_index();
-  const int nk_all = ga.p[0].K / Cfg8<BN>::BK;
+  const Hot x = load_hot(ga);
+  const int t = xcd_chunk_of(x);
+  const int nk_all = x.nk;
   if constexpr (SPLITK) {
-    select_tile<BN>(ga, t >> 1, pi, m0, n0);
-    gemm8_body<EPI, BN, LAY, M16, true>(ga, smem, pi, m0, n0, (t & 1) * (nk_all >> 1), nk_all >> 1, t >> 1, t & 1);
+    select_tile<BN>(x, t >> 1, pi, m0, n0);
+    gemm8_body<EPI, BN, LAY, M16, true>(ga, smem, pi, m0, n0, (t & 1) * (nk_all >> 1), nk_all >> 1, t >> 1, t & 1, &st);
   } else {
-    select_tile<BN>(ga, t, pi, m0, n0);
-    gemm8_body<EPI, BN, LAY, M16>(ga, smem, pi, m0, n0, 0, nk_all, -1);
-  }
+    select_tile<BN>(x, t, pi, m0, n0);
+    gemm8_body<EPI, BN, LAY, M16>(ga, smem, pi, m0, n0, 0, nk_all, -1, 0, &st);
+  }
+  st.mark<4>();
+  st.flush();
 }
 
 struct Cfg10 {
@@ -461,21 +521,24 @@
   const int lane = tid & 63;
   const int wave = __builtin_amdgcn_readfirstlane(tid >> 6);
   const int wm = wave >> 1, wn = wave & 1;
-  const fk_gemm_args& p = ga.p[pi];
-  const BufDesc od_a = make_buf_desc((const bf16_t*)p.A + fk_row_offset(p.a, m0), 0x7fffffffu);
-  const BufDesc od_w = make_buf_desc((const bf16_t*)p.W + (int64_t)n0 * p.ldw, 0x7fffffffu);
+  const ProbEntry q = load_prob(ga, pi);
   const int lrow = lane >> 3, chunk = lane & 7;
   i32x8_t a_voff, w_voff;
+  int64_t a_first;
   {
-    const TileRows arow(p.a, m0);
-    const int ldw2 = (int)p.ldw * 2;
+    const int ldw2 = q.ldw * 2;
+    int rls[8], aoff[8];
+#pragma unroll
+    for (int i = 0; i < 8; ++i) rls[i] = wave * 64 + i * 8 + lrow;
+    a_first = tile_a_rows<8>(ga, pi, q, m0, rls, aoff);
 #pragma unroll
     for (int i = 0; i < 8; ++i) {
-      const int rl = wave * 64 + i * 8 + lrow;
-      a_voff[i] = arow.off(min(rl, p.M - 1 - m0)) * 2 + chunk * 16;
-      w_voff[i] = min(rl, p.N - 1 - n0) * ldw2 + chunk * 16;
-    }
-  }
+      a_voff[i] = aoff[i] * 2 + chunk * 16;
+      w_voff[i] = min(rls[i], q.N - 1 - n0) * ldw2 + chunk * 16;
+    }
+  }
+  const BufDesc od_a = make_buf_desc((const bf16_t*)q.A + a_first, 0x7fffffffu);
+  const BufDesc od_w = make_buf_desc((const bf16_t*)q.W + (int64_t)n0 * q.ldw, 0x7fffffffu);
   const int base = (int)lds_addr_of(smem);
   i32x8_t rd;
   i32x4_t wr;
@@ -570,7 +633,8 @@
 #include "gemm10_loop_x20.inc"
         G10_OPERANDS_X); }
 #endif
-  store_tile<EPI, 256, C>(acc, p, smem, m0, n0, wm, wn);
+  const fk_gemm_args& p = ga.p[behind_requests(pi)];
+  store_tile<EPI, 256, C>(acc, p, smem, m0, n0, wm, wn, nullptr, q.flags);
 #ifdef FK_G10_EXPERIMENTS
   if constexpr (V > 0) {
     if (tid == 0) {
@@ -587,18 +651,19 @@
 template <int EPI, int V = 0, bool PERSIST = false>
 __global__ __launch_bounds__(256, 1) void gemm10_kernel(const GroupArgs ga) {
   extern __shared__ __attribute__((aligned(16))) char smem[];
-  const int nk = ga.p[0].K / Cfg10::BK;
+  const Hot x = load_hot(ga);
+  const int nk = x.nk;
   if constexpr (PERSIST) {
-    const int total = ga.tiles_before[FK_MAX_GROUP];
-    for (int t = xcd_chunk_index(); t < total; t += gridDim.x) {
+    const int total = ga.e.cls[0].before[FK_MAX_GROUP];
+    for (int t = xcd_chunk_of(x); t < total; t += (int)x.grid) {
       int pi, m0, n0;
-      select_tile<256>(ga, t, pi, m0, n0);
+      select_tile<256>(x, t, pi, m0, n0);
       gemm10_body<EPI, V>(ga, smem, pi, m0, n0, 0, nk);
       asm volatile("s_waitcnt lgkmcnt(0)\n\ts_barrier" ::: "memory");
     }
   } else {
     int pi, m0, n0;
-    select_tile<256>(ga, xcd_chunk_index(), pi, m0, n0);
+    select_tile<256>(x, xcd_chunk_of(x), pi, m0, n0);
     gemm10_body<EPI, V>(ga, smem, pi, m0, n0, 0, nk);
   }
 }
@@ -606,9 +671,10 @@
 template <int EPI, int BN, bool M16 = false>
 __global__ __launch_bounds__(512, 2) void gemm8_streamk_kernel(const GroupArgs ga) {
   extern __shared__ __attribute__((aligned(16))) char smem[];
-  const int pos = xcd_chunk_index();
-  const unsigned G = gridDim.x, nk = ga.p[0].K / Cfg8<BN>::BK;
-  const unsigned U = (unsigned)ga.tiles_before[FK_MAX_GROUP] * nk, qU = U / G, rU = U - qU * G;
+  const Hot x = load_hot(ga);
+  const int pos = xcd_chunk_of(x);
+  const unsigned G = x.grid, nk = (unsigned)x.nk;
+  const unsigned U = (unsigned)ga.e.cls[0].before[FK_MAX_GROUP] * nk, qU = U / G, rU = U - qU * G;
   auto cut = [&](unsigned j) __attribute__((always_inline)) {
     unsigned c = qU * j + (rU * j) / G;
     const unsigned r = c % nk;
@@ -623,7 +689,7 @@
     const int k1 = u_end - t * (int)nk, k0 = max(u - t * (int)nk, 0);
     u_end -= k1 - k0;
     int pi, m0, n0;
-    select_tile<BN>(ga, t, pi, m0, n0);
+    select_tile<BN>(x, t, pi, m0, n0);
     const bool part = k0 > 0 || k1 < (int)nk;
     gemm8_body<EPI, BN, 0, M16>(ga, smem, pi, m0, n0, k0, k1 - k0, part ? (k1 < (int)nk ? pos + 1 : pos) : -1);
     __syncthreads();
@@ -631,19 +697,18 @@
 }
 
 template <int BN>
-int count_tiles(GroupArgs& ga, const fk_gemm_args* probs, int n) {
-  int total = 0;
-  for (int i = 0; i < FK_MAX_GROUP; ++i) {
-    ga.tiles_before[i] = total;
-    if (i < n) total += ((probs[i].M + BM - 1) / BM) * ((probs[i].N + BN - 1) / BN);
-  }
-  ga.tiles_before[FK_MAX_GROUP] = total;
+int count_tiles(GroupArgs& ga, const fk_gemm_args* probs, int n, int grid = 0, bool split = false) {
+  int32_t Ms[FK_MAX_GROUP];
+  for (int i = 0; i < n; ++i) Ms[i] = probs[i].M;
+  const int total = tm_fill_class(ga.e.cls[0], Ms, n, (probs[0].N + BN - 1) / BN, 0, ga.e.group_m);
+  if (total >= 0) tm_fill_grid(ga.e, (uint32_t)(grid ? grid : split ? 2 * total : total));
   return total;
 }
 
 template <int EPI, int BN, bool SPLITK, int LAY = 0, bool M16 = false>
 int launch8(GroupArgs& ga, const fk_gemm_args* probs, int n, hipStream_t stream) {
-  const int total = count_tiles<BN>(ga, probs, n);
+  const int total = count_tiles<BN>(ga, probs, n, 0, SPLITK);
+  if (total < 0) return FK_E2BIG_STRIDES;
   auto kern = gemm8_kernel<EPI, BN, SPLITK, LAY, M16>;
   FK_ENSURE_MAX_LDS(kern, Cfg8<BN>::SMEM_BYTES, "fk_gemm_bf16 (256 x 256 tile, 8 waves ping-pong)");
   hipLaunchKernelGGL(kern, dim3(SPLITK ? 2 * total : total), dim3(512), Cfg8<BN>::SMEM_BYTES, stream, ga);
@@ -653,7 +718,7 @@
 
 template <int EPI, int BN, bool M16 = false>
 int launch8_streamk(GroupArgs& ga, const fk_gemm_args* probs, int n, int grid, hipStream_t stream) {
-  count_tiles<BN>(ga, probs, n);
+  if (count_tiles<BN>(ga, probs, n, grid) < 0) return FK_E2BIG_STRIDES;
   auto kern = gemm8_streamk_kernel<EPI, BN, M16>;
   FK_ENSURE_MAX_LDS(kern, Cfg8<BN>::SMEM_BYTES, "fk_gemm_bf16 (256 x 256 tile, stream-K ranges)");
   hipLaunchKernelGGL(kern, dim3(grid), dim3(512), Cfg8<BN>::SMEM_BYTES, stream, ga);
@@ -666,6 +731,7 @@
 template <int EPI>
 int launch10(GroupArgs& ga, const fk_gemm_args* probs, int n, hipStream_t stream) {
   const int total = count_tiles<256>(ga, probs, n);
+  if (total < 0) return FK_E2BIG_STRIDES;
 #ifdef FK_G10_EXPERIMENTS
   if constexpr (EPI == FK_EPI_NONE) {
     static const int x = getenv("FK_G10_X") ? atoi(getenv("FK_G10_X")) : 0;
@@ -697,7 +763,9 @@
     }
     if (kx) {
       if (hipFuncSetAttribute((const void*)kx, hipFuncAttributeMaxDynamicSharedMemorySize, Cfg10::SMEM_BYTES) != hipSuccess) return FK_EINVAL;
-      hipLaunchKernelGGL(kx, dim3(persist ? (total < cu_count() ? total : cu_count()) : total), dim3(256), Cfg10::SMEM_BYTES, stream, ga);
+      const int gx = persist ? (total < cu_count() ? total : cu_count()) : total;
+      tm_fill_grid(ga.e, (uint32_t)gx);
+      hipLaunchKernelGGL(kx, dim3(gx), dim3(256), Cfg10::SMEM_BYTES, stream, ga);
       FK_CHECK_LAUNCH("fk_gemm_bf16 (gemm10 experiment)");
       return FK_OK;
     }
@@ -706,6 +774,7 @@
   const int G = cu_count();
   if (total >= 4 * G) {
     auto kern = gemm10_kernel<EPI, 0, true>;
+    tm_fill_grid(ga.e, (uint32_t)G);
     FK_ENSURE_MAX_LDS(kern, Cfg10::SMEM_BYTES, "fk_gemm_bf16 (256 x 256 tile, 4 waves, hand-placed loop, one workgroup per CU)");
     hipLaunchKernelGGL(kern, dim3(G), dim3(256), Cfg10::SMEM_BYTES, stream, ga);
     FK_CHECK_LAUNCH("fk_gemm_bf16 (256 x 256 tile, 4 waves, hand-placed loop, one workgroup per CU)");
@@ -738,38 +807,40 @@
 };
 
 template <int EPI, int BN, bool M16 = false>
-FK_DEV void gemm9_body(const GroupArgs& ga, char* smem, int pi, int m0, int n0) {
+FK_DEV void gemm9_body(const GroupArgs& ga, char* smem, int pi, int m0, int n0, int nk, EntryStamps* st = nullptr) {
+  EntryStamps st_none;
+  if (!st) st = &st_none;
   using C = Cfg9<BN, M16>;
   const int tid = threadIdx.x;
   const int lane = tid & 63;
   const int wave = __builtin_amdgcn_readfirstlane(tid >> 6);
   const int wm = wave & 3, wn = wave >> 2;
-  const fk_gemm_args& p = ga.p[pi];
-  const int nk = p.K / C::BK;
+  const ProbEntry q = load_prob(ga, pi);
 
   const int lrow = lane >> 3, slot = lane & 7;
-  const __amdgpu_buffer_rsrc_t rs_a =
-      __builtin_amdgcn_make_buffer_rsrc((void*)((const bf16_t*)p.A + fk_row_offset(p.a, m0)), 0, 0x7fffffff, 0x00020000);
-  const __amdgpu_buffer_rsrc_t rs_w =
-      __builtin_amdgcn_make_buffer_rsrc((void*)((const bf16_t*)p.W + (int64_t)n0 * p.ldw), 0, 0x7fffffff, 0x00020000);
   int a_voff[2][2], w_voff[2];
+  int64_t a_first;
   {
-    const TileRows arow(p.a, m0);
-    const int ldw2 = (int)p.ldw * 2;
+    const int ldw2 = q.ldw * 2;
+    int rls[4], aoff[4];
+#pragma unroll
+    for (int i = 0; i < 4; ++i) rls[i] = (i >> 1) * 128 + (wave * 2 + (i & 1)) * 8 + lrow;
+    a_first = tile_a_rows<4>(ga, pi, q, m0, rls, aoff);
 #pragma unroll
     for (int h = 0; h < 2; ++h)
 #pragma unroll
-      for (int j = 0; j < 2; ++j) {
-        const int rl = h * 128 + (wave * 2 + j) * 8 + lrow;
-        a_voff[h][j] = arow.off(min(rl, p.M - 1 - m0)) * 2 + ((slot ^ C::swz(rl)) << 4);
-      }
+      for (int j = 0; j < 2; ++j) a_voff[h][j] = aoff[h * 2 + j] * 2 + ((slot ^ C::swz(rls[h * 2 + j])) << 4);
 #pragma unroll
     for (int j = 0; j < 2; ++j) {
       const int sr = wave * 8 + lrow;
       const int rl = (sr >> 5) * 64 + j * 32 + (sr & 31);
-      w_voff[j] = min(rl, p.N - 1 - n0) * ldw2 + ((slot ^ C::swz(sr)) << 4);
-    }
-  }
+      w_voff[j] = min(rl, q.N - 1 - n0) * ldw2 + ((slot ^ C::swz(sr)) << 4);
+    }
+  }
+  const __amdgpu_buffer_rsrc_t rs_a =
+      __builtin_amdgcn_make_buffer_rsrc((void*)((const bf16_t*)q.A + a_first), 0, 0x7fffffff, 0x00020000);
+  const __amdgpu_buffer_rsrc_t rs_w =
+      __builtin_amdgcn_make_buffer_rsrc((void*)((const bf16_t*)q.W + (int64_t)n0 * q.ldw), 0, 0x7fffffff, 0x00020000);
   auto dma_a = [&](int stage, int kt) {
     const int koff = min(kt, nk - 1) * (C::BK * 2);
     char* dst = smem + stage * C::STAGE_BYTES + wave * 2048;
@@ -782,6 +853,16 @@
     const int koff = min(kt, nk - 1) * (C::BK * 2);
     buffer_lds16(rs_w, smem + stage * C::STAGE_BYTES + 2 * C::A_HALF + j * C::W_PART + wave * 1024, w_voff[j], koff);
   };
+
+  dma_w(0, 0, 0);
+  st->mark<1>();
+  dma_a(0, 0);
+  dma_w(1, 0, 0);
+  dma_w(0, 1, 1);
+  dma_a(1, 1);
+  dma_w(1, 1, 1);
+  dma_w(0, 2, 2);
+  const fk_gemm_args& p = ga.p[behind_requests(pi)];
 
   constexpr int NKS = M16 ? 2 : 4, ASUB = M16 ? 4 : 2, WSUB = M16 ? 2 : 1;
   constexpr int SUB_BYTES = (M16 ? 16 : 32) * C::ROW_BYTES;
@@ -840,13 +921,6 @@
   using V10 = std::integral_constant<int, 10>;
   using V8 = std::integral_constant<int, 8>;
 
-  dma_w(0, 0, 0);
-  dma_a(0, 0);
-  dma_w(1, 0, 0);
-  dma_w(0, 1, 1);
-  dma_a(1, 1);
-  dma_w(1, 1, 1);
-  dma_w(0, 2, 2);
   wait_vmcnt<8>();
   __builtin_amdgcn_sched_barrier(0);
   __builtin_amdgcn_s_barrier();
@@ -854,6 +928,7 @@
   read_w(0, 0);
   if (wn == 1) __builtin_amdgcn_s_barrier();
   __builtin_amdgcn_sched_barrier(0);
+  st->mark<2>();
 
   auto tile_body = [&](auto sc, int kt) {
     constexpr int st = decltype(sc)::value, st1 = (st + 1) % 3, st2 = (st + 2) % 3;
@@ -865,23 +940,30 @@
     if (kt + 1 < nk) tile_body(std::integral_constant<int, 1>{}, kt + 1);
     if (kt + 2 < nk) tile_body(std::integral_constant<int, 2>{}, kt + 2);
   }
+  st->mark<3>();
   if (wn == 0) __builtin_amdgcn_s_barrier();
   asm volatile("s_waitcnt vmcnt(0)" ::: "memory");
 
-  store_tile<EPI, BN, C>(acc, p, smem, m0, n0, wm, wn);
+  store_tile<EPI, BN, C>(acc, p, smem, m0, n0, wm, wn, nullptr, q.flags);
 }
 
 template <int EPI, int BN, bool M16 = false>
 __global__ __launch_bounds__(512, 2) void gemm9_kernel(const GroupArgs ga) {
   extern __shared__ __attribute__((aligned(16))) char smem[];
+  EntryStamps st;
+  st.mark<0>();
   int pi, m0, n0;
-  select_tile<BN>(ga, xcd_chunk_index(), pi, m0, n0);
-  gemm9_body<EPI, BN, M16>(ga, smem, pi, m0, n0);
+  const Hot x = load_hot(ga);
+  select_tile<BN>(x, xcd_chunk_of(x), pi, m0, n0);
+  gemm9_body<EPI, BN, M16>(ga, smem, pi, m0, n0, x.nk, &st);
+  st.mark<4>();
+  st.flush();
 }
 
 template <int EPI, int BN, bool M16 = false>
 int launch9(GroupArgs& ga, const fk_gemm_args* probs, int n, hipStream_t stream) {
   const int total = count_tiles<BN>(ga, probs, n);
+  if (total < 0) return FK_E2BIG_STRIDES;
   auto kern = gemm9_kernel<EPI, BN, M16>;
   FK_ENSURE_MAX_LDS(kern, Cfg9<BN>::SMEM_BYTES, "fk_gemm_bf16 (256 x 128 tile, 8 waves ping-pong)");
   hipLaunchKernelGGL(kern, dim3(total), dim3(512), Cfg9<BN>::SMEM_BYTES, stream, ga);
@@ -892,17 +974,27 @@
 template <int EPI, bool M16 = false>
 __global__ __launch_bounds__(512, 2) void gemm_mix_kernel(const GroupArgs ga) {
   extern __shared__ __attribute__((aligned(16))) char smem[];
+  EntryStamps st;
+  st.mark<0>();
   const int xcd = blockIdx.x & 7, idx = blockIdx.x >> 3;
-  const int nbig = ga.xcd_big_cnt[xcd];
+  Hot x;
+  x.h = tm_hot(ga.e, ga.e.cls[0]);
+  TmHot hs = tm_hot(ga.e, ga.e.cls[1]);
+  x.xq = ga.e.xq; x.xr = ga.e.xr; x.grid = ga.e.grid; x.nk = ga.e.nk;
+  const TileEntry::Xcd tab = ga.e.xcd[xcd];
+  int nbig = tab.big_cnt, big0 = tab.big_start, small0 = tab.small_start;
+  asm volatile("" : FK_PIN_HEAD(x), "+s"(nbig), "+s"(big0), "+s"(small0), FK_PIN_CLASS(x.h), FK_PIN_CLASS(hs));
   int pi, m0, n0;
   if (idx < nbig) {
-    tile_of<256>(ga, ga.tiles_before, ga.xcd_big_start[xcd] + idx, ga.big_cols, 0, pi, m0, n0);
-    gemm8_body<EPI, 256, 0, M16>(ga, smem, pi, m0, n0, 0, ga.p[0].K / 64, -1);
+    tm_tile_hot(x.h, 256, big0 + idx, pi, m0, n0);
+    gemm8_body<EPI, 256, 0, M16>(ga, smem, pi, m0, n0, 0, x.nk, -1, 0, &st);
   } else {
-    tile_of<128>(ga, ga.small_before, ga.xcd_small_start[xcd] + idx - nbig, (ga.p[0].N - ga.big_cols * 256 + 127) / 128,
-                 ga.big_cols * 256, pi, m0, n0);
-    gemm9_body<EPI, 128, M16>(ga, smem, pi, m0, n0);
-  }
+    hs.n = x.h.n; hs.group_m = x.h.group_m;
+    tm_tile_hot(hs, 128, small0 + idx - nbig, pi, m0, n0);
+    gemm9_body<EPI, 128, M16>(ga, smem, pi, m0, n0, x.nk, &st);
+  }
+  st.mark<4>();
+  st.flush();
 }
 
 constexpr int MIX_SMEM = Cfg8<256>::SMEM_BYTES > Cfg9<128>::SMEM_BYTES ? Cfg8<256>::SMEM_BYTES : Cfg9<128>::SMEM_BYTES;
@@ -910,30 +1002,21 @@
 template <int EPI, bool M16 = false>
 int launch_mix(GroupArgs& ga, const fk_gemm_args* probs, int n, int big_cols, hipStream_t stream) {
   const int ncols128 = (probs[0].N - big_cols * 256 + 127) / 128;
-  int tb = 0, ts = 0;
-  for (int i = 0; i < FK_MAX_GROUP; ++i) {
-    ga.tiles_before[i] = tb;
-    ga.small_before[i] = ts;
-    if (i < n) {
-      const int nbm = (probs[i].M + BM - 1) / BM;
-      tb += nbm * big_cols;
-      ts += nbm * ncols128;
-    }
-  }
-  ga.tiles_before[FK_MAX_GROUP] = tb;
-  ga.small_before[FK_MAX_GROUP] = ts;
-  ga.big_cols = big_cols;
+  int32_t Ms[FK_MAX_GROUP];
+  for (int i = 0; i < n; ++i) Ms[i] = probs[i].M;
+  const int tb = tm_fill_class(ga.e.cls[0], Ms, n, big_cols, 0, ga.e.group_m);
+  const int ts = tm_fill_class(ga.e.cls[1], Ms, n, ncols128, big_cols * 256, ga.e.group_m);
+  if (tb < 0 || ts < 0) return FK_E2BIG_STRIDES;
   const int W = tb + ts;
   int bs = 0, ss = 0;
   for (int x = 0; x < 8; ++x) {
     const int wx = W / 8 + (x < W % 8 ? 1 : 0), bx = tb / 8 + (x < tb % 8 ? 1 : 0);
     if (wx < bx) return FK_E2BIG_STRIDES;
-    ga.xcd_big_start[x] = bs;
-    ga.xcd_big_cnt[x] = bx;
-    ga.xcd_small_start[x] = ss;
+    ga.e.xcd[x] = {bs, bx, ss, 0};
     bs += bx;
     ss += wx - bx;
   }
+  tm_fill_grid(ga.e, (uint32_t)W);
   auto kern = gemm_mix_kernel<EPI, M16>;
   FK_ENSURE_MAX_LDS(kern, MIX_SMEM, "fk_gemm_bf16 (mixed 256 x 256 / 256 x 128 tiles)");
   hipLaunchKernelGGL(kern, dim3(W), dim3(512), MIX_SMEM, stream, ga);
@@ -1061,9 +1144,14 @@
                       : sk_bits == FK_GEMM_PLAN_SPLITK_UNANNOUNCED ? SK_SYM_UNANNOUNCED : SK_MODE_DEFAULT;
   GroupArgs ga;
   ga.sk_mode = sk_mode;
-  ga.n = n;
-  ga.group_m = ctl.group_m ? ctl.group_m : GROUP_M;
-  ga.big_cols = 0;
+  ga.e = TileEntry{};
+  ga.e.n = n;
+  ga.e.nk = probs[0].K / 64;
+  {
+    int32_t Ms[FK_MAX_GROUP];
+    for (int i = 0; i < n; ++i) Ms[i] = probs[i].M;
+    ga.e.group_m = tm_group_m(Ms, n, ctl.group_m ? ctl.group_m : GROUP_M);
+  }
   ga.sk_partials = nullptr;
   ga.sk_ctl = nullptr;
   long nbm_total = 0;
@@ -1087,6 +1175,23 @@
     }
   }
   if (!ok32) return FK_E2BIG_STRIDES;
+  for (int i = 0; i < FK_MAX_GROUP; ++i) {
+    const fk_gemm_args& q = ga.p[i];
+    ProbEntry& e = ga.pe[i];
+    e.A = q.A;
+    e.W = q.W;
+    e.lda = (int32_t)q.a.ld;
+    e.ldw = (int32_t)q.ldw;
+    e.M = q.M;
+    e.N = q.N;
+    e.K = q.K;
+    e.flags = 0;
+    if (tm_rows_flat(q.a.ld, q.a.rows_per_batch, q.a.batch_stride, q.M)) e.flags |= TM_A_FLAT;
+    if (q.epilogue == FK_EPI_QKV ? (q.c.rows_per_batch > 0 && q.M <= q.c.rows_per_batch)
+                                 : tm_rows_flat(q.c.ld, q.c.rows_per_batch, q.c.batch_stride, q.M)) e.flags |= TM_C_FLAT;
+    if (tm_rows_flat(q.r.ld, q.r.rows_per_batch, q.r.batch_stride, q.M)) e.flags |= TM_R_FLAT;
+    if (q.gate_rows_per_batch <= 0 || q.M <= q.gate_rows_per_batch) e.flags |= TM_G_FLAT;
+  }
 
   const int lay = probs[0].layout;
   if (lay != 0) {
@@ -1171,9 +1276,17 @@
     case FK_EPI_QKV: rc = launch_variant<FK_EPI_QKV>(ga, probs, n, plan.variant, plan.big_cols, m16, stream); break;
     default: fk_set_error("fk_gemm_bf16: unknown epilogue %d", probs[0].epilogue); return FK_EUNSUPPORTED;
   }
+  if (rc == FK_E2BIG_STRIDES && plan.variant != 384) report_variant(probs, 0);
   if (rc == FK_E2BIG_STRIDES && plan.variant == 384) {
     report_variant(probs, 128);
     return fk_gemm2_launch(probs, n, 128, stream);
   }
   return rc;
 }
+
+#ifdef FK_ENTRY_STAMPS
+extern "C" int fk_entry_stamps_set(void* buf) {
+  unsigned long long* p = (unsigned long long*)buf;
+  return hipMemcpyToSymbol(HIP_SYMBOL(fk_entry_stamp_buf), &p, sizeof(p)) == hipSuccess ? 0 : -1;
+}
+#endif
diff --git a/gpt_image_edit_amd/csrc/gemm_tile_map.h b/gpt_image_edit_amd/csrc/gemm_tile_map.h
--- /dev/null
+++ b/gpt_image_edit_amd/csrc/gemm_tile_map.h
@@ -0,0 +1,137 @@
+#pragma once
+#include <stdint.h>
+
+#ifndef FK_TM_FN
+#define FK_TM_FN inline
+#endif
+#if defined(__clang__)
+#define TM_UNROLL _Pragma("unroll")
+#else
+#define TM_UNROLL
+#endif
+
+constexpr int TM_MAX_GROUP = 4;
+constexpr int TM_BM = 256;
+
+FK_TM_FN uint32_t tm_magic(uint32_t d) { return (uint32_t)(((1ull << 31) + d - 1) / d); }
+FK_TM_FN uint32_t tm_div(uint32_t t, uint32_t magic) { return (uint32_t)(((uint64_t)(t << 1) * magic) >> 32); }
+FK_TM_FN bool tm_div_domain(uint64_t t_max, uint64_t d) { return d >= 1 && t_max < (1ull << 31) && t_max * d <= (1ull << 31); }
+
+struct TmClass {
+  int32_t before[TM_MAX_GROUP + 1];
+  int32_t per_group, col0;
+  uint32_t per_group_mul, group_m_mul;
+  int32_t nbm[TM_MAX_GROUP];
+  uint32_t last_mul[TM_MAX_GROUP];
+};
+
+struct TileEntry {
+  uint32_t grid, xq, xr;
+  int32_t n, group_m, nk;
+  TmClass cls[2];
+  struct Xcd { int32_t big_start, big_cnt, small_start, pad_; } xcd[8];
+};
+
+enum { TM_A_FLAT = 1, TM_C_FLAT = 2, TM_R_FLAT = 4, TM_G_FLAT = 8 };
+struct ProbEntry {
+  const void* A;
+  const void* W;
+  int32_t lda, ldw;
+  int32_t M, N, K;
+  int32_t flags;
+};
+
+FK_TM_FN bool tm_rows_flat(int64_t ld, int64_t rows_per_batch, int64_t batch_stride, int64_t M) {
+  return rows_per_batch <= 0 || M <= rows_per_batch || batch_stride == rows_per_batch * ld;
+}
+
+FK_TM_FN int tm_xcd_chunk(uint32_t xq, uint32_t xr, uint32_t bid) {
+  const uint32_t xcd = bid & 7, idx = bid >> 3;
+  return (int)((xcd < xr ? xcd * (xq + 1) : xr * (xq + 1) + (xcd - xr) * xq) + idx);
+}
+FK_TM_FN int tm_xcd_chunk(const TileEntry& e, uint32_t bid) { return tm_xcd_chunk(e.xq, e.xr, bid); }
+
+struct TmHot {
+  int32_t n, group_m;
+  int32_t before[TM_MAX_GROUP - 1];
+  int32_t nbm[TM_MAX_GROUP];
+  uint32_t last_mul[TM_MAX_GROUP];
+  int32_t per_group, col0;
+  uint32_t per_group_mul, group_m_mul;
+};
+FK_TM_FN TmHot tm_hot(const TileEntry& e, const TmClass& c) {
+  TmHot h;
+  h.n = e.n;
+  h.group_m = e.group_m;
+  TM_UNROLL
+  for (int i = 0; i < TM_MAX_GROUP; ++i) {
+    if (i > 0) h.before[i - 1] = c.before[i];
+    h.nbm[i] = c.nbm[i];
+    h.last_mul[i] = c.last_mul[i];
+  }
+  h.per_group = c.per_group;
+  h.col0 = c.col0;
+  h.per_group_mul = c.per_group_mul;
+  h.group_m_mul = c.group_m_mul;
+  return h;
+}
+
+FK_TM_FN void tm_tile_hot(const TmHot& h, int bn, int t, int& pi, int& m0, int& n0) {
+  pi = 0;
+  int base = 0, nbm = h.nbm[0];
+  uint32_t lmul = h.last_mul[0];
+  TM_UNROLL
+  for (int i = 1; i < TM_MAX_GROUP; ++i) {
+    const bool here = i < h.n && t >= h.before[i - 1];
+    pi = here ? i : pi;
+    base = here ? h.before[i - 1] : base;
+    nbm = here ? h.nbm[i] : nbm;
+    lmul = here ? h.last_mul[i] : lmul;
+  }
+  const uint32_t u = (uint32_t)(t - base);
+  const uint32_t g = tm_div(u, h.per_group_mul);
+  const int first_m = (int)g * h.group_m;
+  const bool full = nbm - first_m >= h.group_m;
+  const int gm = full ? h.group_m : nbm - first_m;
+  const uint32_t rem = u - g * (uint32_t)h.per_group;
+  const uint32_t col = tm_div(rem, full ? h.group_m_mul : lmul);
+  m0 = (first_m + (int)(rem - col * (uint32_t)gm)) * TM_BM;
+  n0 = h.col0 + (int)col * bn;
+}
+FK_TM_FN void tm_tile(const TileEntry& e, const TmClass& c, int bn, int t, int& pi, int& m0, int& n0) {
+  tm_tile_hot(tm_hot(e, c), bn, t, pi, m0, n0);
+}
+
+FK_TM_FN int tm_group_m(const int32_t* M, int n, int group_m) {
+  int deepest = 1;
+  for (int i = 0; i < n; ++i) {
+    const int nbm = (M[i] + TM_BM - 1) / TM_BM;
+    if (nbm > deepest) deepest = nbm;
+  }
+  return group_m < deepest ? group_m : deepest;
+}
+
+FK_TM_FN int tm_fill_class(TmClass& c, const int32_t* M, int n, int nbn, int col0, int group_m) {
+  int total = 0;
+  for (int i = 0; i < TM_MAX_GROUP; ++i) {
+    c.before[i] = total;
+    const int nbm = i < n ? (M[i] + TM_BM - 1) / TM_BM : 0;
+    c.nbm[i] = nbm;
+    const int last = nbm > 0 ? nbm - ((nbm - 1) / group_m) * group_m : 1;
+    c.last_mul[i] = tm_magic((uint32_t)last);
+    total += nbm * nbn;
+  }
+  c.before[TM_MAX_GROUP] = total;
+  c.col0 = col0;
+  c.per_group = group_m * nbn;
+  c.per_group_mul = tm_magic((uint32_t)c.per_group);
+  c.group_m_mul = tm_magic((uint32_t)group_m);
+  if (!tm_div_domain((uint64_t)total, (uint64_t)c.per_group) || !tm_div_domain((uint64_t)c.per_group, (uint64_t)group_m)) return -1;
+  return total;
+}
+
+FK_TM_FN void tm_fill_grid(TileEntry& e, uint32_t grid) {
+  e.grid = grid;
+  e.xq = grid >> 3;
+  e.xr = grid & 7;
+}
```

After: 1.093 images/s, median of 6. 1.01x the previous value.
